# William-wAng618/roboticAttack

Hardware: AMD Instinct MI355X
Metric: attack-steps/sec (bs=64, 3x50x50 patch, OpenVLA-7B) (higher is better)
Workload: dtype bf16; 1 GPU; UADA_wrapper_ddp inner step: bs=64/rank (global 64), patch 3,50,50, geometry=True, maskidx=[0]; OpenVLA-7B shape, random init; u8 frames resident in HBM; global_batch=64, parallelism=dp1, regions=weak, visible_gpus=1, labelled_rows_per_rank=128, tunableop_entries_loaded_min_over_ranks=173

## Files before the change

include/vaa_model_ops.h:

```cpp
#ifndef VAA_MODEL_OPS_H_
#define VAA_MODEL_OPS_H_
#include <stdint.h>
#ifdef __cplusplus
extern "C" {
#endif
int vaa_model_rope(const uint16_t* x, long sb, long st, long sh, const float* cos_t, const float* sin_t, int B, int T, int H, int hd,
                   float sin_sign, uint16_t* out, void* stream);
int vaa_model_swiglu_fwd(const uint16_t* gate, const uint16_t* up, uint16_t* y, long n, void* stream);
int vaa_model_swiglu_bwd(const uint16_t* dy, const uint16_t* gate, const uint16_t* up, uint16_t* dgate, uint16_t* dup, long n, void* stream);
int vaa_model_scale_add(const uint16_t* x, const uint16_t* a, const uint16_t* ls, uint16_t* out, long rows, int D, void* stream);
int vaa_model_rmsnorm_fwd(const uint16_t* x, const uint16_t* w, uint16_t* h, float* rstd, long rows, int D, float eps, void* stream);
int vaa_model_rmsnorm_bwd(const uint16_t* gh, const uint16_t* gpass, const uint16_t* x, const uint16_t* w, const float* rstd, uint16_t* gx,
                          long rows, int D, void* stream);
int vaa_model_layernorm_fwd(const uint16_t* x, const uint16_t* w, const uint16_t* b, uint16_t* h, float* stats, long rows, int D, float eps,
                            void* stream);
int vaa_model_layernorm_bwd(const uint16_t* gh, const uint16_t* gpass, const uint16_t* x, const uint16_t* w, const float* stats, uint16_t* gx,
                            long rows, int D, void* stream);
int vaa_model_attention_fwd(const uint16_t* q, const int64_t* q_str, const uint16_t* k, const int64_t* k_str, const uint16_t* v,
                            const int64_t* v_str, uint16_t* o, const int64_t* o_str, float* lse, const int32_t* cu_seqlens, int B, int H,
                            int T, int hd, int causal, float scale, void* stream);
int vaa_model_attention_bwd(const uint16_t* q, const int64_t* q_str, const uint16_t* k, const int64_t* k_str, const uint16_t* v,
                            const int64_t* v_str, const uint16_t* o, const int64_t* o_str, const uint16_t* dout, const int64_t* do_str,
                            const float* lse, float* dsum, uint16_t* dq, const int64_t* dq_str, uint16_t* dk, const int64_t* dk_str,
                            uint16_t* dv, const int64_t* dv_str, const float* rope_cos, const float* rope_sin, const int32_t* cu_seqlens, int B,
                            int H, int T, int hd, int causal, float scale, void* stream);
#ifdef __cplusplus
}
#endif
#endif
```

roboticattack_amd/_lib.py:

```python
from __future__ import annotations

import ctypes as C
import os

_HERE = os.path.dirname(os.path.abspath(__file__))
LIB_PATH = os.environ.get("VAA_LIB_PATH") or os.path.join(_HERE, "libvaa_hip.so")

VAA_OK = 0
MASK_LT_M20, MASK_NE_M100 = 0, 1
LOSS_UADA, LOSS_UADA_DDP, LOSS_UPA, LOSS_CE = 0, 1, 2, 3
DTYPE_F32, DTYPE_BF16 = 0, 1
LAYOUT_FULL, LAYOUT_ROWS = 0, 1
GRAD_FULL, GRAD_SLICE = 0, 1
OPT_ADAMW_HF, OPT_PGD_SIGN = 0, 1

MODEL_OP_EXPORTS = ("vaa_model_rope", "vaa_model_swiglu_fwd", "vaa_model_swiglu_bwd", "vaa_model_rmsnorm_fwd", "vaa_model_rmsnorm_bwd",
                    "vaa_model_attention_fwd", "vaa_model_attention_bwd", "vaa_model_layernorm_fwd", "vaa_model_layernorm_bwd", "vaa_model_scale_add")

EXPORTS = (
    "vaa_last_error",
    "vaa_version",
    "vaa_device_check",
    "vaa_patch_apply_fwd",
    "vaa_patch_grad_ws_bytes",
    "vaa_patch_grad_gather",
    "vaa_loss_ws_bytes",
    "vaa_loss_fwd_bwd",
    "vaa_loss_fwd_bwd_ex",
    "vaa_patch_update",
    "vaa_patch_apply_eval",
    "vaa_patch_embed_grad_ws_bytes",
    "vaa_patch_embed_grad_gather",
    "vaa_patch_embed_packed_elems",
    "vaa_patch_embed_pack_weights",
    "vaa_patch_embed_grad_multi_ws_bytes",
    "vaa_patch_embed_grad_gather_multi",
    "vaa_patch_resize_fwd",
    "vaa_patch_resize_ws_bytes",
    "vaa_patch_resize_bwd",
    "vaa_patch_apply_fwd_multi",
    "vaa_patch_grad_gather_multi",
    "vaa_loss_rowmap_bytes",
    "vaa_loss_rowmap_build",
    "vaa_loss_rows_ws_bytes",
    "vaa_loss_rows_fwd_bwd",
    "vaa_patch_apply_fwd_tiles",
    "vaa_patch_grad_partials",
    "vaa_patch_embed_grad_gather_multi_tiles",
    "vaa_patch_embed_grad_gather_tiles",
    "vaa_loss_rows_stats",
    "vaa_head_loss_ws_bytes",
    "vaa_head_loss_rows_applies",
    "vaa_head_loss_rows_stats",
    "vaa_head_loss_rows_finish",
    "vaa_head_slice_applies",
    "vaa_head_slice_ws_bytes",
    "vaa_head_slice_pack",
    "vaa_head_slice_fwd_bwd",
    "vaa_step_epilogue",
    "vaa_step_epilogue_update",
    "vaa_loss_rowmap_seg_bytes",
    "vaa_loss_rowmap_build_seg",
    "vaa_step_epilogue_seg",
    "vaa_step_epilogue_seg_update",
    "vaa_patch_update_seg",
    "vaa_async_error",
    "vaa_prof_start",
    "vaa_prof_stop",
    "vaa_prof_get",
)


class VaaError(RuntimeError):
    pass


_lib = None


def _up_to_date() -> bool:
    if not os.path.exists(LIB_PATH):
        return False
    t = os.path.getmtime(LIB_PATH)
    src = os.path.join(_HERE, "csrc")
    deps = [os.path.join(src, f) for f in os.listdir(src)] + [os.path.join(_HERE, "..", "include", f) for f in ("vaa.h", "vaa_model_ops.h")]
    return all(os.path.getmtime(d) <= t for d in deps if os.path.exists(d))


def build(verbose: bool = False, force: bool = True) -> str:
    import fcntl
    import subprocess

    script = os.path.join(_HERE, "csrc", "build.sh")
    with open(os.path.join(_HERE, ".build.lock"), "w") as lock:
        fcntl.flock(lock, fcntl.LOCK_EX)
        try:
            if not force and _up_to_date():
                return LIB_PATH
            out = subprocess.run(["bash", script], capture_output=True, text=True)
        finally:
            fcntl.flock(lock, fcntl.LOCK_UN)
    if out.returncode != 0:
        raise VaaError(f"building libvaa_hip.so failed:\n{out.stdout}\n{out.stderr}")
    if verbose:
        print(out.stdout.strip())
    return LIB_PATH


def lib() -> C.CDLL:
    global _lib
    if _lib is not None:
        return _lib
    if not os.path.exists(LIB_PATH) and not os.environ.get("VAA_LIB_PATH") and os.path.exists(os.environ.get("HIPCC", "/opt/rocm/bin/hipcc")):
        build(force=False)
    if not os.path.exists(LIB_PATH):
        raise VaaError(
            f"{LIB_PATH} not found: the HIP extension is required (no CPU fallback). "
            "Build it with `python -c 'import __graft_entry__ as g; g.build()'` or roboticattack_amd/csrc/build.sh"
        )
    try:
        import torch
    except Exception:
        pass
    L = C.CDLL(LIB_PATH)
    vp, i32, f32, sz = C.c_void_p, C.c_int, C.c_float, C.c_size_t
    L.vaa_last_error.restype = C.c_char_p
    L.vaa_last_error.argtypes = []
    L.vaa_version.restype = i32
    L.vaa_device_check.restype = i32
    L.vaa_patch_apply_fwd.restype = i32
    L.vaa_patch_apply_fwd.argtypes = [vp, vp, vp, vp, i32, i32, i32, i32, i32, C.POINTER(f32), C.POINTER(f32), vp, vp, vp]
    L.vaa_patch_grad_ws_bytes.restype = sz
    L.vaa_patch_grad_ws_bytes.argtypes = [i32, i32, i32]
    L.vaa_patch_grad_gather.restype = i32
    L.vaa_patch_grad_gather.argtypes = [vp, vp, vp, vp, vp, i32, i32, i32, i32, i32, C.POINTER(f32), vp, vp, sz, vp]
    L.vaa_patch_embed_grad_ws_bytes.restype = sz
    L.vaa_patch_embed_grad_ws_bytes.argtypes = [i32, i32, i32]
    L.vaa_patch_embed_packed_elems.restype = sz
    L.vaa_patch_embed_packed_elems.argtypes = [i32]
    L.vaa_patch_embed_pack_weights.restype = i32
    L.vaa_patch_embed_pack_weights.argtypes = [vp, i32, vp, vp]
    L.vaa_patch_embed_grad_gather.restype = i32
    L.vaa_patch_embed_grad_gather.argtypes = [vp, i32, vp, i32, vp, vp, vp, vp, vp, vp, i32, i32, i32, i32, i32, C.POINTER(f32), i32, vp, vp, sz, vp]
    L.vaa_patch_embed_grad_multi_ws_bytes.restype = sz
    L.vaa_patch_embed_grad_multi_ws_bytes.argtypes = [i32]
    L.vaa_patch_embed_grad_gather_multi.restype = i32
    L.vaa_patch_embed_grad_gather_multi.argtypes = [vp, i32, vp, i32, vp, vp, vp, vp, vp, vp, vp, i32, i32, i32, i32, i32, C.POINTER(f32), i32, vp, vp, sz, vp]
    L.vaa_patch_resize_fwd.restype = i32
    L.vaa_patch_resize_fwd.argtypes = [vp, i32, i32, vp, i32, vp, vp]
    L.vaa_patch_resize_ws_bytes.restype = sz
    L.vaa_patch_resize_ws_bytes.argtypes = [i32, i32, i32]
    L.vaa_patch_resize_bwd.restype = i32
    L.vaa_patch_resize_bwd.argtypes = [vp, i32, i32, vp, i32, vp, vp, sz, vp]
    L.vaa_patch_apply_fwd_multi.restype = i32
    L.vaa_patch_apply_fwd_multi.argtypes = [vp, vp, vp, vp, vp, i32, i32, i32, i32, i32, C.POINTER(f32), C.POINTER(f32), vp, vp, vp]
    L.vaa_patch_grad_gather_multi.restype = i32
    L.vaa_patch_grad_gather_multi.argtypes = [vp, vp, vp, vp, vp, vp, i32, i32, i32, i32, i32, C.POINTER(f32), vp, vp]
    L.vaa_loss_ws_bytes.restype = sz
    L.vaa_loss_ws_bytes.argtypes = [i32, i32]
    L.vaa_loss_fwd_bwd.restype = i32
    L.vaa_loss_fwd_bwd.argtypes = [vp, i32, i32, vp, i32, i32, i32, i32, i32, C.POINTER(f32), vp, vp, vp, vp, sz, vp]
    L.vaa_loss_fwd_bwd_ex.restype = i32
    L.vaa_loss_fwd_bwd_ex.argtypes = [vp, i32, i32, vp, i32, i32, i32, i32, i32, C.POINTER(f32), vp, vp, vp, vp, vp, sz, vp]
    L.vaa_loss_rowmap_bytes.restype = sz
    L.vaa_loss_rowmap_bytes.argtypes = [i32, i32]
    L.vaa_loss_rowmap_build.restype = i32
    L.vaa_loss_rowmap_build.argtypes = [vp, i32, i32, vp, sz, vp]
    L.vaa_loss_rows_ws_bytes.restype = sz
    L.vaa_loss_rows_ws_bytes.argtypes = [i32]
    L.vaa_loss_rows_fwd_bwd.restype = i32
    L.vaa_loss_rows_fwd_bwd.argtypes = [vp, i32, vp, i32, i32, i32, i32, i32, C.POINTER(f32), vp, vp, vp, vp, i32, vp, sz, vp]
    L.vaa_patch_update.restype = i32
    L.vaa_patch_update.argtypes = [vp, vp, vp, vp, i32, i32, f32, f32, f32, f32, i32, f32, f32, vp, vp]
    L.vaa_patch_apply_eval.restype = i32
    L.vaa_patch_apply_eval.argtypes = [vp, vp, vp, vp, vp, i32, i32, i32, vp, vp]
    L.vaa_patch_apply_fwd_tiles.restype = i32
    L.vaa_patch_apply_fwd_tiles.argtypes = [vp, vp, vp, vp, vp, i32, i32, i32, i32, i32, C.POINTER(f32), C.POINTER(f32), vp, vp, vp, vp, vp]
    L.vaa_patch_embed_grad_gather_multi_tiles.restype = i32
    L.vaa_patch_embed_grad_gather_multi_tiles.argtypes = [vp, i32, vp, i32, vp, vp, vp, vp, vp, vp, vp, vp, i32, i32, i32, i32, i32, C.POINTER(f32), i32, vp, vp, sz, vp]
    L.vaa_patch_grad_partials.restype = i32
    L.vaa_patch_grad_partials.argtypes = [i32]
    L.vaa_patch_embed_grad_gather_tiles.restype = i32
    L.vaa_patch_embed_grad_gather_tiles.argtypes = [vp, i32, vp, i32, vp, vp, vp, vp, vp, vp, vp, i32, i32, i32, i32, i32, C.POINTER(f32), i32, vp, vp, sz, vp]
    L.vaa_loss_rows_stats.restype = i32
    L.vaa_loss_rows_stats.argtypes = [vp, i32, vp, i32, i32, i32, i32, i32, C.POINTER(f32), vp, i32, vp, sz, vp]
    L.vaa_head_loss_ws_bytes.restype = sz
    L.vaa_head_loss_ws_bytes.argtypes = [i32, i32]
    L.vaa_head_loss_rows_applies.restype = i32
    L.vaa_head_loss_rows_applies.argtypes = [i32, i32, i32]
    L.vaa_head_loss_rows_stats.restype = i32
    L.vaa_head_loss_rows_stats.argtypes = [vp, vp, i32, vp, i32, i32, i32, i32, i32, C.POINTER(f32), vp, vp, sz, vp, sz, vp, vp]
    L.vaa_head_loss_rows_finish.restype = i32
    L.vaa_head_loss_rows_finish.argtypes = [vp, i32, i32, i32, i32, i32, C.POINTER(f32), vp, sz, vp, sz, vp, vp, vp, vp, vp]
    L.vaa_head_slice_applies.restype = i32
    L.vaa_head_slice_applies.argtypes = [i32, i32, i32]
    L.vaa_head_slice_ws_bytes.restype = sz
    L.vaa_head_slice_ws_bytes.argtypes = [i32]
    L.vaa_head_slice_pack.restype = i32
    L.vaa_head_slice_pack.argtypes = [vp, i32, i32, vp, vp]
    L.vaa_head_slice_fwd_bwd.restype = i32
    L.vaa_head_slice_fwd_bwd.argtypes = [vp, vp, vp, i32, vp, i32, i32, i32, i32, i32, C.POINTER(f32), vp, vp, vp, sz, vp, vp, vp, vp, sz, vp]
    L.vaa_step_epilogue.restype = i32
    L.vaa_step_epilogue.argtypes = [vp, i32, i32, vp, i32, i32, i32, i32, i32, C.POINTER(f32), vp, sz, vp, vp, vp, vp, vp]
    L.vaa_step_epilogue_update.restype = i32
    L.vaa_step_epilogue_update.argtypes = [vp, i32, i32, vp, i32, i32, i32, i32, i32, C.POINTER(f32), vp, sz, vp, vp, vp, vp, vp, vp, vp, i32, f32, f32, f32, f32,
                                           i32, vp, vp]
    L.vaa_loss_rowmap_seg_bytes.restype = sz
    L.vaa_loss_rowmap_seg_bytes.argtypes = [i32, i32, i32]
    L.vaa_loss_rowmap_build_seg.restype = i32
    L.vaa_loss_rowmap_build_seg.argtypes = [vp, i32, i32, i32, vp, sz, vp]
    L.vaa_step_epilogue_seg.restype = i32
    L.vaa_step_epilogue_seg.argtypes = [vp, i32, i32, i32, vp, i32, i32, i32, i32, i32, C.POINTER(f32), vp, sz, vp, vp, vp, vp, vp]
    L.vaa_step_epilogue_seg_update.restype = i32
    L.vaa_step_epilogue_seg_update.argtypes = [vp, i32, i32, i32, vp, i32, i32, i32, i32, i32, C.POINTER(f32), vp, sz, vp, vp, vp, vp, vp, vp, vp, i32, f32,
                                               f32, f32, f32, i32, vp, vp]
    L.vaa_patch_update_seg.restype = i32
    L.vaa_patch_update_seg.argtypes = [vp, vp, vp, vp, i32, i32, i32, f32, f32, f32, f32, i32, f32, f32, vp, vp]
    L.vaa_async_error.restype = i32
    L.vaa_async_error.argtypes = []
    L.vaa_prof_start.restype = i32
    L.vaa_prof_start.argtypes = [i32]
    L.vaa_prof_stop.restype = i32
    L.vaa_prof_stop.argtypes = []
    L.vaa_prof_get.restype = i32
    L.vaa_prof_get.argtypes = [i32, C.POINTER(C.c_char_p), C.POINTER(f32)]
    lng = C.c_long
    L.vaa_model_rope.restype = i32
    L.vaa_model_rope.argtypes = [vp, lng, lng, lng, vp, vp, i32, i32, i32, i32, f32, vp, vp]
    L.vaa_model_swiglu_fwd.restype = i32
    L.vaa_model_swiglu_fwd.argtypes = [vp, vp, vp, lng, vp]
    L.vaa_model_swiglu_bwd.restype = i32
    L.vaa_model_swiglu_bwd.argtypes = [vp, vp, vp, vp, vp, lng, vp]
    L.vaa_model_scale_add.restype = i32
    L.vaa_model_scale_add.argtypes = [vp, vp, vp, vp, lng, i32, vp]
    L.vaa_model_rmsnorm_fwd.restype = i32
    L.vaa_model_rmsnorm_fwd.argtypes = [vp, vp, vp, vp, lng, i32, f32, vp]
    L.vaa_model_rmsnorm_bwd.restype = i32
    L.vaa_model_rmsnorm_bwd.argtypes = [vp, vp, vp, vp, vp, vp, lng, i32, vp]
    L.vaa_model_layernorm_fwd.restype = i32
    L.vaa_model_layernorm_fwd.argtypes = [vp, vp, vp, vp, vp, lng, i32, f32, vp]
    L.vaa_model_layernorm_bwd.restype = i32
    L.vaa_model_layernorm_bwd.argtypes = [vp, vp, vp, vp, vp, vp, lng, i32, vp]
    i64p = C.POINTER(C.c_int64)
    L.vaa_model_attention_fwd.restype = i32
    L.vaa_model_attention_fwd.argtypes = [vp, i64p, vp, i64p, vp, i64p, vp, i64p, vp, vp, i32, i32, i32, i32, i32, f32, vp]
    L.vaa_model_attention_bwd.restype = i32
    L.vaa_model_attention_bwd.argtypes = [vp, i64p, vp, i64p, vp, i64p, vp, i64p, vp, i64p, vp, vp, vp, i64p, vp, i64p, vp, i64p, vp, vp, vp, i32, i32, i32, i32, i32, f32, vp]
    _lib = L
    return L


def check(rc: int, what: str) -> None:
    if rc != VAA_OK:
        msg = lib().vaa_last_error().decode("utf-8", "replace")
        raise VaaError(f"{what} failed with code {rc}: {msg}")


def f32x(vals):
    return (C.c_float * len(vals))(*[float(v) for v in vals])
```

roboticattack_amd/csrc/vaa_attention.hip:

```cpp
#include "vaa_common.h"

#include <cstdlib>
#include <mutex>

#include "../../include/vaa_model_ops.h"

namespace vaa {

typedef short v4s __attribute__((ext_vector_type(4)));
typedef short v8s __attribute__((ext_vector_type(8)));
typedef float v4f __attribute__((ext_vector_type(4)));
typedef __attribute__((address_space(3))) v4s* lds_v4s_ptr;

struct AttnStr {
    long b, t, h;
};

struct AttnFwdArgs {
    const uint16_t *q, *k, *v;
    uint16_t* o;
    float* lse;
    AttnStr sq, sk, sv, so;
    const int32_t* cu;
    int B, H, T, hd;
    float scale_log2;
};

struct SeqInfo {
    int T;
    long tok0;
    bool packed;
};
__device__ __forceinline__ SeqInfo seq_info(const int32_t* cu, int b, int Tmax) {
    SeqInfo si;
    si.packed = cu != nullptr;
    si.tok0 = si.packed ? cu[b] : 0;
    si.T = si.packed ? cu[b + 1] - cu[b] : Tmax;
    return si;
}
__device__ __forceinline__ long row_base(const AttnStr& st, const SeqInfo& si, int b, int h) {
    return (si.packed ? si.tok0 * st.t : (long)b * st.b) + (long)h * st.h;
}

constexpr int kTile = 64;

__device__ __forceinline__ float fast_exp2(float x) { return __builtin_amdgcn_exp2f(x); }

__device__ __forceinline__ v4s lds_tr16(const uint16_t* p) {
    return __builtin_amdgcn_ds_read_tr16_b64_v4i16((lds_v4s_ptr)(p));
}

__device__ __forceinline__ v8s cat8(v4s lo, v4s hi) { return __builtin_shufflevector(lo, hi, 0, 1, 2, 3, 4, 5, 6, 7); }

typedef __bf16 bf2 __attribute__((ext_vector_type(2)));
typedef float f2 __attribute__((ext_vector_type(2)));

__device__ __forceinline__ uint32_t cvt_pk_bf16(float lo, float hi) {
    const bf2 r = __builtin_convertvector((f2){lo, hi}, bf2);
    return *reinterpret_cast<const uint32_t*>(&r);
}

__device__ __forceinline__ v8s pack8(v4f a, v4f b) {
    uint4 r;
    r.x = cvt_pk_bf16(a[0], a[1]);
    r.y = cvt_pk_bf16(a[2], a[3]);
    r.z = cvt_pk_bf16(b[0], b[1]);
    r.w = cvt_pk_bf16(b[2], b[3]);
    return *reinterpret_cast<v8s*>(&r);
}

typedef unsigned int v4u __attribute__((ext_vector_type(4)));

__device__ __forceinline__ __amdgpu_buffer_rsrc_t slice_rsrc(const uint16_t* base, long st, int T, int hd) {
    return __builtin_amdgcn_make_buffer_rsrc((void*)base, 0, (int)((((long)T - 1) * st + hd) * 2), 0x00020000);
}

template <int HDP>
struct TileRegs {
    static constexpr int kChunks = kTile * (HDP / 8) / 256;
    v4u r[kChunks];
    __device__ __forceinline__ void load(__amdgpu_buffer_rsrc_t rs, int st_bytes, int row0) {
#pragma unroll
        for (int it = 0; it < kChunks; ++it) {
            const int ch = threadIdx.x + it * 256;
            const int row = ch / (HDP / 8), cc = ch % (HDP / 8);
            r[it] = __builtin_amdgcn_raw_buffer_load_b128(rs, (row0 + row) * st_bytes + cc * 16, 0, 0);
        }
    }
    __device__ __forceinline__ void store(uint16_t* lds, int stride) const {
#pragma unroll
        for (int it = 0; it < kChunks; ++it) {
            const int ch = threadIdx.x + it * 256;
            const int row = ch / (HDP / 8), cc = ch % (HDP / 8);
            *reinterpret_cast<v4u*>(lds + row * stride + cc * 8) = r[it];
        }
    }
};

__device__ __forceinline__ bool block_to_pair(int nblk, int npairs, int& pair, int& blk, bool late_first = true) {
    const int bid = blockIdx.x, xcd = bid & 7, slot = bid >> 3;
    pair = (slot / nblk) * 8 + xcd;
    blk = late_first ? nblk - 1 - (slot % nblk) : slot % nblk;
    return pair < npairs;
}

template <int KS, int NT, bool CAUSAL, int G>
__global__ __launch_bounds__(256) void attn_fwd_kernel(AttnFwdArgs a) {
    constexpr int HDP = KS * 32;
    constexpr int SK = HDP + 8;
    constexpr int SV = HDP + 16;
    constexpr int QB = kTile * G, QW = 16 * G;
    __shared__ __attribute__((aligned(16))) uint16_t sK[kTile * SK];
    __shared__ __attribute__((aligned(16))) uint16_t sV[kTile * SV];

    const int nqb = (a.T + QB - 1) / QB;
    int pair, qb;
    if (!block_to_pair(nqb, a.B * a.H, pair, qb)) return;
    const int b = pair / a.H, h = pair - b * a.H;
    const SeqInfo si = seq_info(a.cu, b, a.T);
    const int T = si.T;
    if (qb * QB >= T) return;
    const int tid = threadIdx.x, lane = tid & 63, wv = tid >> 6, c = lane & 15, g = lane >> 4;
    const int q0 = qb * QB + wv * QW;

    const uint16_t* qp = a.q + row_base(a.sq, si, b, h);
    const uint16_t* kp = a.k + row_base(a.sk, si, b, h);
    const uint16_t* vp = a.v + row_base(a.sv, si, b, h);

    v8s qf[G][KS];
#pragma unroll
    for (int j = 0; j < G; ++j) {
        const int q = q0 + 16 * j + c;
#pragma unroll
        for (int ks = 0; ks < KS; ++ks) {
            const int d0 = ks * 32 + g * 8;
            uint4 r = make_uint4(0, 0, 0, 0);
            if (q < T && d0 < a.hd) r = *reinterpret_cast<const uint4*>(qp + (long)q * a.sq.t + d0);
            qf[j][ks] = *reinterpret_cast<v8s*>(&r);
        }
    }

    const int kend = CAUSAL ? min(T, (qb + 1) * QB) : T;
    const int ntile = (kend + kTile - 1) / kTile;

    v4f acc[G][NT];
    float m[G], lsum[G];
#pragma unroll
    for (int j = 0; j < G; ++j) {
#pragma unroll
        for (int nt = 0; nt < NT; ++nt) acc[j][nt] = (v4f){0.f, 0.f, 0.f, 0.f};
        m[j] = -INFINITY;
        lsum[j] = 0.0f;
    }

    const __amdgpu_buffer_rsrc_t krs = slice_rsrc(kp, a.sk.t, T, a.hd), vrs = slice_rsrc(vp, a.sv.t, T, a.hd);
    const int kst = (int)a.sk.t * 2, vst = (int)a.sv.t * 2;
    TileRegs<HDP> rk, rv;
    rk.load(krs, kst, 0);
    rv.load(vrs, vst, 0);
    for (int kt = 0; kt < ntile; ++kt) {
        __syncthreads();
        rk.store(sK, SK);
        rv.store(sV, SV);
        __syncthreads();
        if (kt + 1 < ntile) {
            rk.load(krs, kst, (kt + 1) * kTile);
            rv.load(vrs, vst, (kt + 1) * kTile);
        }
        const int key0 = kt * kTile;
        if (CAUSAL && key0 > q0 + QW - 1) continue;

        v4f st[G][4];
#pragma unroll
        for (int rp = 0; rp < 2; ++rp) {
            v8s kfr[2][KS];
#pragma unroll
            for (int rl = 0; rl < 2; ++rl)
#pragma unroll
                for (int ks = 0; ks < KS; ++ks) kfr[rl][ks] = *reinterpret_cast<const v8s*>(&sK[((2 * rp + rl) * 16 + c) * SK + ks * 32 + g * 8]);
#pragma unroll
            for (int j = 0; j < G; ++j)
#pragma unroll
                for (int rl = 0; rl < 2; ++rl) {
                    v4f t = (v4f){0.f, 0.f, 0.f, 0.f};
#pragma unroll
                    for (int ks = 0; ks < KS; ++ks) t = __builtin_amdgcn_mfma_f32_16x16x32_bf16(kfr[rl][ks], qf[j][ks], t, 0, 0, 0);
                    st[j][2 * rp + rl] = t;
                }
        }
#pragma unroll
        for (int j = 0; j < G; ++j) {
            const int qj0 = q0 + 16 * j, q = qj0 + c;
            const bool need_mask = (key0 + kTile > T) || (CAUSAL && key0 + kTile - 1 > qj0);
            if (need_mask) {
#pragma unroll
                for (int rt = 0; rt < 4; ++rt)
#pragma unroll
                    for (int r = 0; r < 4; ++r) {
                        const int key = key0 + rt * 16 + g * 4 + r;
                        if (key >= T || (CAUSAL && key > q)) st[j][rt][r] = -INFINITY;
                    }
            }
            float mx = -INFINITY;
#pragma unroll
            for (int rt = 0; rt < 4; ++rt)
#pragma unroll
                for (int r = 0; r < 4; ++r) mx = fmaxf(mx, st[j][rt][r]);
            mx = fmaxf(mx, __shfl_xor(mx, 16, 64));
            mx = fmaxf(mx, __shfl_xor(mx, 32, 64));
            const float mn = fmaxf(m[j], mx * a.scale_log2);
            const float mu = (mn == -INFINITY) ? 0.0f : mn;
            const float alpha = fast_exp2(m[j] - mu);
            m[j] = mn;
            float ps = 0.0f;
#pragma unroll
            for (int rt = 0; rt < 4; ++rt)
#pragma unroll
                for (int r = 0; r < 4; ++r) {
                    const float p = fast_exp2(__builtin_fmaf(st[j][rt][r], a.scale_log2, -mu));
                    st[j][rt][r] = p;
                    ps += p;
                }
            lsum[j] = lsum[j] * alpha + ps;
#pragma unroll
            for (int nt = 0; nt < NT; ++nt) acc[j][nt] *= alpha;
        }
#pragma unroll
        for (int half = 0; half < 2; ++half) {
            const uint16_t* vrow = &sV[(half * 32 + 4 * g + (c >> 2)) * SV + (c & 3) * 4];
            v8s vfr[NT];
#pragma unroll
            for (int nt = 0; nt < NT; ++nt) vfr[nt] = cat8(lds_tr16(vrow + nt * 16), lds_tr16(vrow + 16 * SV + nt * 16));
#pragma unroll
            for (int j = 0; j < G; ++j) {
                const v8s pf = pack8(st[j][2 * half], st[j][2 * half + 1]);
#pragma unroll
                for (int nt = 0; nt < NT; ++nt) acc[j][nt] = __builtin_amdgcn_mfma_f32_16x16x32_bf16(vfr[nt], pf, acc[j][nt], 0, 0, 0);
            }
        }
    }
#pragma unroll
    for (int j = 0; j < G; ++j) {
        const int q = q0 + 16 * j + c;
        float ls = lsum[j];
        ls += __shfl_xor(ls, 16, 64);
        ls += __shfl_xor(ls, 32, 64);
        if (q < T) {
            const float inv = ls > 0.0f ? 1.0f / ls : 0.0f;
            uint16_t* op = a.o + row_base(a.so, si, b, h) + (long)q * a.so.t;
#pragma unroll
            for (int nt = 0; nt < NT; ++nt) {
                const int d0 = nt * 16 + g * 4;
                if (d0 < a.hd) {
                    uint2 w;
                    w.x = cvt_pk_bf16(acc[j][nt][0] * inv, acc[j][nt][1] * inv);
                    w.y = cvt_pk_bf16(acc[j][nt][2] * inv, acc[j][nt][3] * inv);
                    *reinterpret_cast<uint2*>(op + d0) = w;
                }
            }
            if (g == 0) a.lse[((long)b * a.H + h) * a.T + q] = (m[j] + __builtin_log2f(ls)) * 0.69314718055994531f;
        }
    }
}

struct AttnBwdArgs {
    const uint16_t *q, *k, *v, *o, *dout;
    const float* lse;
    float* dsum;
    uint16_t *dq, *dk, *dv;
    AttnStr sq, sk, sv, so, sdo, sdq, sdk, sdv;
    const int32_t* cu;
    const float *rope_cos, *rope_sin;
    int B, H, T, hd;
    float scale, scale_log2;
};

template <int NT>
__device__ __forceinline__ void store_grad_row(uint16_t* op, const v4f (&acc)[NT], float scale, int g, int hd, const float* cosr, const float* sinr) {
    if (cosr) {
#pragma unroll
        for (int nt = 0; nt < NT / 2; ++nt) {
            const int d0 = nt * 16 + g * 4;
            const float4 c4 = *reinterpret_cast<const float4*>(cosr + d0), s4 = *reinterpret_cast<const float4*>(sinr + d0);
            const float cs[4] = {c4.x, c4.y, c4.z, c4.w}, sn[4] = {s4.x, s4.y, s4.z, s4.w};
            float o1[4], o2[4];
#pragma unroll
            for (int r = 0; r < 4; ++r) {
                const float g1 = acc[nt][r] * scale, g2 = acc[nt + NT / 2][r] * scale;
                o1[r] = g1 * cs[r] + g2 * sn[r];
                o2[r] = g2 * cs[r] - g1 * sn[r];
            }
            uint2 w;
            w.x = cvt_pk_bf16(o1[0], o1[1]); w.y = cvt_pk_bf16(o1[2], o1[3]);
            *reinterpret_cast<uint2*>(op + d0) = w;
            w.x = cvt_pk_bf16(o2[0], o2[1]); w.y = cvt_pk_bf16(o2[2], o2[3]);
            *reinterpret_cast<uint2*>(op + d0 + NT * 8) = w;
        }
        return;
    }
#pragma unroll
    for (int nt = 0; nt < NT; ++nt) {
        const int d0 = nt * 16 + g * 4;
        if (d0 < hd) {
            uint2 w;
            w.x = cvt_pk_bf16(acc[nt][0] * scale, acc[nt][1] * scale);
            w.y = cvt_pk_bf16(acc[nt][2] * scale, acc[nt][3] * scale);
            *reinterpret_cast<uint2*>(op + d0) = w;
        }
    }
}

template <int KS>
__device__ __forceinline__ void load_row_frags(v8s (&f)[KS], const uint16_t* row, bool valid, int g, int hd) {
#pragma unroll
    for (int ks = 0; ks < KS; ++ks) {
        const int d0 = ks * 32 + g * 8;
        uint4 r = make_uint4(0, 0, 0, 0);
        if (valid && d0 < hd) r = *reinterpret_cast<const uint4*>(row + d0);
        f[ks] = *reinterpret_cast<v8s*>(&r);
    }
}

__device__ __forceinline__ float bf_lo(uint32_t w) { return __uint_as_float(w << 16); }
__device__ __forceinline__ float bf_hi(uint32_t w) { return __uint_as_float(w & 0xffff0000u); }

template <int KS>
__device__ __forceinline__ void load_tile_frags(v8s (&af)[KS], const uint16_t* tile, int stride, int rt, int c, int g) {
#pragma unroll
    for (int ks = 0; ks < KS; ++ks) af[ks] = *reinterpret_cast<const v8s*>(&tile[(rt * 16 + c) * stride + ks * 32 + g * 8]);
}
template <int KS>
__device__ __forceinline__ v4f frag_dot(const v8s (&af)[KS], const v8s (&bf)[KS]) {
    v4f acc = (v4f){0.f, 0.f, 0.f, 0.f};
#pragma unroll
    for (int ks = 0; ks < KS; ++ks) acc = __builtin_amdgcn_mfma_f32_16x16x32_bf16(af[ks], bf[ks], acc, 0, 0, 0);
    return acc;
}

template <int KS, int NT, bool CAUSAL, int G>
__global__ __launch_bounds__(256) void attn_bwd_dq_kernel(AttnBwdArgs a) {
    constexpr int HDP = KS * 32;
    constexpr int SK = HDP + 16, SV = HDP + 8;
    constexpr int QB = kTile * G, QW = 16 * G;
    __shared__ __attribute__((aligned(16))) uint16_t sK[kTile * SK];
    __shared__ __attribute__((aligned(16))) uint16_t sV[kTile * SV];

    const int nqb = (a.T + QB - 1) / QB;
    int pair, qb;
    if (!block_to_pair(nqb, a.B * a.H, pair, qb)) return;
    const int b = pair / a.H, h = pair - b * a.H;
    const SeqInfo si = seq_info(a.cu, b, a.T);
    const int T = si.T;
    if (qb * QB >= T) return;
    const int tid = threadIdx.x, lane = tid & 63, wv = tid >> 6, c = lane & 15, g = lane >> 4;
    const int q0 = qb * QB + wv * QW;

    const uint16_t* kp = a.k + row_base(a.sk, si, b, h);
    const uint16_t* vp = a.v + row_base(a.sv, si, b, h);
    v8s qf[G][KS], dof[G][KS];
    float Dq[G], lse2[G];
#pragma unroll
    for (int j = 0; j < G; ++j) {
        const int q = q0 + 16 * j + c;
        const bool qv = q < T;
        load_row_frags<KS>(qf[j], a.q + row_base(a.sq, si, b, h) + (long)q * a.sq.t, qv, g, a.hd);
        load_row_frags<KS>(dof[j], a.dout + row_base(a.sdo, si, b, h) + (long)q * a.sdo.t, qv, g, a.hd);
        float dq_ = 0.0f;
        v8s of[KS];
        load_row_frags<KS>(of, a.o + row_base(a.so, si, b, h) + (long)q * a.so.t, qv, g, a.hd);
#pragma unroll
        for (int ks = 0; ks < KS; ++ks)
#pragma unroll
            for (int e = 0; e < 8; ++e) dq_ += bf16_bits_to_f32((uint16_t)of[ks][e]) * bf16_bits_to_f32((uint16_t)dof[j][ks][e]);
        dq_ += __shfl_xor(dq_, 16, 64);
        dq_ += __shfl_xor(dq_, 32, 64);
        Dq[j] = dq_;
        const long rowid = ((long)b * a.H + h) * a.T + q;
        if (qv && g == 0) a.dsum[rowid] = dq_;
        lse2[j] = qv ? a.lse[rowid] * 1.4426950408889634f : INFINITY;
    }

    const int kend = CAUSAL ? min(T, (qb + 1) * QB) : T;
    const int ntile = (kend + kTile - 1) / kTile;
    v4f acc[G][NT];
#pragma unroll
    for (int j = 0; j < G; ++j)
#pragma unroll
        for (int nt = 0; nt < NT; ++nt) acc[j][nt] = (v4f){0.f, 0.f, 0.f, 0.f};

    const __amdgpu_buffer_rsrc_t krs = slice_rsrc(kp, a.sk.t, T, a.hd), vrs = slice_rsrc(vp, a.sv.t, T, a.hd);
    const int kst = (int)a.sk.t * 2, vst = (int)a.sv.t * 2;
    TileRegs<HDP> rk, rv;
    rk.load(krs, kst, 0);
    rv.load(vrs, vst, 0);
    for (int kt = 0; kt < ntile; ++kt) {
        __syncthreads();
        rk.store(sK, SK);
        rv.store(sV, SV);
        __syncthreads();
        if (kt + 1 < ntile) {
            rk.load(krs, kst, (kt + 1) * kTile);
            rv.load(vrs, vst, (kt + 1) * kTile);
        }
        const int key0 = kt * kTile;
        if (CAUSAL && key0 > q0 + QW - 1) continue;
        const bool need_mask = (key0 + kTile > T) || (CAUSAL && key0 + kTile - 1 > q0);
#pragma unroll
        for (int half = 0; half < 2; ++half) {
            if (CAUSAL && key0 + half * 32 > q0 + QW - 1) continue;
            v4f ds[G][2];
#pragma unroll
            for (int rl = 0; rl < 2; ++rl) {
                const int rt = 2 * half + rl;
                v8s ak[KS], av[KS];
                load_tile_frags<KS>(ak, sK, SK, rt, c, g);
                load_tile_frags<KS>(av, sV, SV, rt, c, g);
#pragma unroll
                for (int j = 0; j < G; ++j) {
                    const v4f st = frag_dot<KS>(ak, qf[j]);
                    const v4f dp = frag_dot<KS>(av, dof[j]);
                    const int q = q0 + 16 * j + c;
#pragma unroll
                    for (int r = 0; r < 4; ++r) {
                        float p = fast_exp2(__builtin_fmaf(st[r], a.scale_log2, -lse2[j]));
                        if (need_mask) {
                            const int key = key0 + rt * 16 + g * 4 + r;
                            if (key >= T || (CAUSAL && key > q)) p = 0.0f;
                        }
                        ds[j][rl][r] = p * (dp[r] - Dq[j]);
                    }
                }
            }
            const uint16_t* krow = &sK[(half * 32 + 4 * g + (c >> 2)) * SK + (c & 3) * 4];
            v8s kfr[NT];
#pragma unroll
            for (int nt = 0; nt < NT; ++nt) kfr[nt] = cat8(lds_tr16(krow + nt * 16), lds_tr16(krow + 16 * SK + nt * 16));
#pragma unroll
            for (int j = 0; j < G; ++j) {
                const v8s dsf = pack8(ds[j][0], ds[j][1]);
#pragma unroll
                for (int nt = 0; nt < NT; ++nt) acc[j][nt] = __builtin_amdgcn_mfma_f32_16x16x32_bf16(kfr[nt], dsf, acc[j][nt], 0, 0, 0);
            }
        }
    }
#pragma unroll
    for (int j = 0; j < G; ++j) {
        const int q = q0 + 16 * j + c;
        if (q < T) {
            const long ro = (si.tok0 + q) * (a.hd >> 1);
            store_grad_row<NT>(a.dq + row_base(a.sdq, si, b, h) + (long)q * a.sdq.t, acc[j], a.scale, g, a.hd,
                               a.rope_cos ? a.rope_cos + ro : nullptr, a.rope_cos ? a.rope_sin + ro : nullptr);
        }
    }
}

template <int KS, int NT, bool CAUSAL, int G>
__global__ __launch_bounds__(256) void attn_bwd_dkv_kernel(AttnBwdArgs a) {
    constexpr int HDP = KS * 32;
    constexpr int SQ = HDP + 16;
    constexpr int KB = kTile * G, KW = 16 * G;
    __shared__ __attribute__((aligned(16))) uint16_t sQ[kTile * SQ];
    __shared__ __attribute__((aligned(16))) uint16_t sDO[kTile * SQ];
    __shared__ float sL[kTile], sD[kTile];

    const int nkb = (a.T + KB - 1) / KB;
    int pair, kb;
    if (!block_to_pair(nkb, a.B * a.H, pair, kb, !CAUSAL)) return;
    const int b = pair / a.H, h = pair - b * a.H;
    const SeqInfo si = seq_info(a.cu, b, a.T);
    const int T = si.T;
    if (kb * KB >= T) return;
    const int tid = threadIdx.x, lane = tid & 63, wv = tid >> 6, c = lane & 15, g = lane >> 4;
    const int key0w = kb * KB + wv * KW;

    v8s kf[G][KS], vf[G][KS];
#pragma unroll
    for (int j = 0; j < G; ++j) {
        const int key = key0w + 16 * j + c;
        load_row_frags<KS>(kf[j], a.k + row_base(a.sk, si, b, h) + (long)key * a.sk.t, key < T, g, a.hd);
        load_row_frags<KS>(vf[j], a.v + row_base(a.sv, si, b, h) + (long)key * a.sv.t, key < T, g, a.hd);
    }
    const uint16_t* qp = a.q + row_base(a.sq, si, b, h);
    const uint16_t* dop = a.dout + row_base(a.sdo, si, b, h);
    const float* lsep = a.lse + ((long)b * a.H + h) * a.T;
    const float* dsp = a.dsum + ((long)b * a.H + h) * a.T;

    v4f dk[G][NT], dv[G][NT];
#pragma unroll
    for (int j = 0; j < G; ++j)
#pragma unroll
        for (int nt = 0; nt < NT; ++nt) {
            dk[j][nt] = (v4f){0.f, 0.f, 0.f, 0.f};
            dv[j][nt] = (v4f){0.f, 0.f, 0.f, 0.f};
        }
    const int nqt = (T + kTile - 1) / kTile;
    const int qt0 = CAUSAL ? kb * G : 0;
    TileRegs<HDP> rq, rdo;
    float rstat = 0.0f;
    auto load_stats = [&](int qbase) {
        if (tid < 128) {
            const int qq = qbase + (tid & 63);
            if (tid < 64) rstat = qq < T ? lsep[qq] * 1.4426950408889634f : INFINITY;
            else rstat = qq < T ? dsp[qq] : 0.0f;
        }
    };
    const __amdgpu_buffer_rsrc_t qrs = slice_rsrc(qp, a.sq.t, T, a.hd), dors = slice_rsrc(dop, a.sdo.t, T, a.hd);
    const int qst = (int)a.sq.t * 2, dost = (int)a.sdo.t * 2;
    rq.load(qrs, qst, qt0 * kTile);
    rdo.load(dors, dost, qt0 * kTile);
    load_stats(qt0 * kTile);
    for (int qt = qt0; qt < nqt; ++qt) {
        __syncthreads();
        rq.store(sQ, SQ);
        rdo.store(sDO, SQ);
        if (tid < 64) sL[tid] = rstat;
        else if (tid < 128) sD[tid - 64] = rstat;
        __syncthreads();
        if (qt + 1 < nqt) {
            rq.load(qrs, qst, (qt + 1) * kTile);
            rdo.load(dors, dost, (qt + 1) * kTile);
            load_stats((qt + 1) * kTile);
        }
        const int qb0 = qt * kTile;
        if (CAUSAL && qb0 + kTile - 1 < key0w) continue;
        const bool need_mask = CAUSAL && qb0 < key0w + KW - 1;
#pragma unroll
        for (int half = 0; half < 2; ++half) {
            if (CAUSAL && qb0 + half * 32 + 31 < key0w) continue;
            v4f p[G][2], ds[G][2];
#pragma unroll
            for (int rl = 0; rl < 2; ++rl) {
                const int rt = 2 * half + rl;
                v8s aq[KS], ado[KS];
                load_tile_frags<KS>(aq, sQ, SQ, rt, c, g);
                load_tile_frags<KS>(ado, sDO, SQ, rt, c, g);
#pragma unroll
                for (int j = 0; j < G; ++j) {
                    const v4f s = frag_dot<KS>(aq, kf[j]);
                    const v4f dp = frag_dot<KS>(ado, vf[j]);
                    const int key = key0w + 16 * j + c;
#pragma unroll
                    for (int r = 0; r < 4; ++r) {
                        const int ql = rt * 16 + g * 4 + r;
                        float pe = fast_exp2(__builtin_fmaf(s[r], a.scale_log2, -sL[ql]));
                        if (CAUSAL && need_mask && key > qb0 + ql) pe = 0.0f;
                        p[j][rl][r] = pe;
                        ds[j][rl][r] = pe * (dp[r] - sD[ql]);
                    }
                }
            }
            const int ro = (half * 32 + 4 * g + (c >> 2)) * SQ + (c & 3) * 4;
            {
                v8s fr[NT];
#pragma unroll
                for (int nt = 0; nt < NT; ++nt) fr[nt] = cat8(lds_tr16(&sDO[ro + nt * 16]), lds_tr16(&sDO[ro + 16 * SQ + nt * 16]));
#pragma unroll
                for (int j = 0; j < G; ++j) {
                    const v8s pf = pack8(p[j][0], p[j][1]);
#pragma unroll
                    for (int nt = 0; nt < NT; ++nt) dv[j][nt] = __builtin_amdgcn_mfma_f32_16x16x32_bf16(fr[nt], pf, dv[j][nt], 0, 0, 0);
                }
#pragma unroll
                for (int nt = 0; nt < NT; ++nt) fr[nt] = cat8(lds_tr16(&sQ[ro + nt * 16]), lds_tr16(&sQ[ro + 16 * SQ + nt * 16]));
#pragma unroll
                for (int j = 0; j < G; ++j) {
                    const v8s dsf = pack8(ds[j][0], ds[j][1]);
#pragma unroll
                    for (int nt = 0; nt < NT; ++nt) dk[j][nt] = __builtin_amdgcn_mfma_f32_16x16x32_bf16(fr[nt], dsf, dk[j][nt], 0, 0, 0);
                }
            }
        }
    }
#pragma unroll
    for (int j = 0; j < G; ++j) {
        const int key = key0w + 16 * j + c;
        if (key < T) {
            const long ro = (si.tok0 + key) * (a.hd >> 1);
            store_grad_row<NT>(a.dk + row_base(a.sdk, si, b, h) + (long)key * a.sdk.t, dk[j], a.scale, g, a.hd,
                               a.rope_cos ? a.rope_cos + ro : nullptr, a.rope_cos ? a.rope_sin + ro : nullptr);
            store_grad_row<NT>(a.dv + row_base(a.sdv, si, b, h) + (long)key * a.sdv.t, dv[j], 1.0f, g, a.hd, nullptr, nullptr);
        }
    }
}

static void attn_groups(int hd, int& gf, int& gq, int& gk) {
    static int cfg[3] = {0, 0, 0};
    static std::once_flag once;
    std::call_once(once, [] {
        const char* ev = getenv("VAA_ATTN_G");
        for (int i = 0; i < 3; ++i) cfg[i] = (ev && ev[0] && ev[1] && ev[2] && (ev[i] == '1' || ev[i] == '2')) ? ev[i] - '0' : 0;
    });
    const int dflt = (hd > 64 && hd <= 80) ? 2 : 1;
    gf = cfg[0] ? cfg[0] : dflt;
    gq = cfg[1] ? cfg[1] : dflt;
    gk = cfg[2] ? cfg[2] : dflt;
}

template <bool CAUSAL>
static int launch_bwd(const AttnBwdArgs& a, hipStream_t st) {
    int gf, gq, gk;
    attn_groups(a.hd, gf, gq, gk);
    const unsigned pairs8 = (unsigned)(((long)a.B * a.H + 7) / 8 * 8);
    const unsigned grid_q = pairs8 * (unsigned)((a.T + kTile * gq - 1) / (kTile * gq)), grid_k = pairs8 * (unsigned)((a.T + kTile * gk - 1) / (kTile * gk));
#define VAA_ATT_BWD(KS, NT)                                                                                                  \
    do {                                                                                                                     \
        if (gq == 2) hipLaunchKernelGGL((attn_bwd_dq_kernel<KS, NT, CAUSAL, 2>), dim3(grid_q), dim3(256), 0, st, a);         \
        else hipLaunchKernelGGL((attn_bwd_dq_kernel<KS, NT, CAUSAL, 1>), dim3(grid_q), dim3(256), 0, st, a);                 \
        int rc = check_launch("vaa_model_attention_bwd(dq)");                                                                \
        if (rc != VAA_OK) return rc;                                                                                         \
        if (gk == 2) hipLaunchKernelGGL((attn_bwd_dkv_kernel<KS, NT, CAUSAL, 2>), dim3(grid_k), dim3(256), 0, st, a);        \
        else hipLaunchKernelGGL((attn_bwd_dkv_kernel<KS, NT, CAUSAL, 1>), dim3(grid_k), dim3(256), 0, st, a);                \
        return check_launch("vaa_model_attention_bwd(dkv)");                                                                 \
    } while (0)
    if (a.hd <= 64) VAA_ATT_BWD(2, 4);
    else if (a.hd <= 80) VAA_ATT_BWD(3, 5);
    else if (a.hd <= 96) VAA_ATT_BWD(3, 6);
    else VAA_ATT_BWD(4, 8);
#undef VAA_ATT_BWD
}

template <bool CAUSAL>
static int launch_fwd(const AttnFwdArgs& a, hipStream_t st) {
    int gf, gq, gk;
    attn_groups(a.hd, gf, gq, gk);
    const unsigned grid = (unsigned)(((long)a.B * a.H + 7) / 8 * 8) * (unsigned)((a.T + kTile * gf - 1) / (kTile * gf));
#define VAA_ATT_FWD(KS, NT)                                                                                          \
    do {                                                                                                             \
        if (gf == 2) hipLaunchKernelGGL((attn_fwd_kernel<KS, NT, CAUSAL, 2>), dim3(grid), dim3(256), 0, st, a);      \
        else hipLaunchKernelGGL((attn_fwd_kernel<KS, NT, CAUSAL, 1>), dim3(grid), dim3(256), 0, st, a);              \
    } while (0)
    if (a.hd <= 64) VAA_ATT_FWD(2, 4);
    else if (a.hd <= 80) VAA_ATT_FWD(3, 5);
    else if (a.hd <= 96) VAA_ATT_FWD(3, 6);
    else VAA_ATT_FWD(4, 8);
#undef VAA_ATT_FWD
    return check_launch("vaa_model_attention_fwd");
}

static bool strides_ok(const int64_t* s) { return s && (s[0] % 8) == 0 && (s[1] % 8) == 0 && (s[2] % 8) == 0; }
static AttnStr mk(const int64_t* s) { AttnStr r; r.b = s[0]; r.t = s[1]; r.h = s[2]; return r; }

}

extern "C" int vaa_model_attention_fwd(const uint16_t* q, const int64_t* q_str, const uint16_t* k, const int64_t* k_str, const uint16_t* v,
                                       const int64_t* v_str, uint16_t* o, const int64_t* o_str, float* lse, const int32_t* cu_seqlens, int B,
                                       int H, int T, int hd, int causal, float scale, void* stream) {
    using namespace vaa;
    if (!q || !k || !v || !o || !lse) {
        set_error("vaa_model_attention_fwd: null pointer argument");
        return VAA_E_INVALID;
    }
    if (B <= 0 || H <= 0 || T <= 0 || hd <= 0 || hd > 128 || (hd % 8) != 0 || !strides_ok(q_str) || !strides_ok(k_str) || !strides_ok(v_str) ||
        !strides_ok(o_str)) {
        set_error("vaa_model_attention_fwd: unsupported shape (B=%d H=%d T=%d hd=%d; hd %% 8 == 0, hd <= 128, strides %% 8 == 0)", B, H, T, hd);
        return VAA_E_UNSUPPORTED;
    }
    AttnFwdArgs a;
    a.q = q; a.k = k; a.v = v; a.o = o; a.lse = lse;
    a.sq = mk(q_str); a.sk = mk(k_str); a.sv = mk(v_str); a.so = mk(o_str);
    a.cu = cu_seqlens;
    a.B = B; a.H = H; a.T = T; a.hd = hd;
    a.scale_log2 = scale * 1.4426950408889634f;
    return causal ? launch_fwd<true>(a, (hipStream_t)stream) : launch_fwd<false>(a, (hipStream_t)stream);
}

extern "C" int vaa_model_attention_bwd(const uint16_t* q, const int64_t* q_str, const uint16_t* k, const int64_t* k_str, const uint16_t* v,
                                       const int64_t* v_str, const uint16_t* o, const int64_t* o_str, const uint16_t* dout,
                                       const int64_t* do_str, const float* lse, float* dsum, uint16_t* dq, const int64_t* dq_str, uint16_t* dk,
                                       const int64_t* dk_str, uint16_t* dv, const int64_t* dv_str, const float* rope_cos, const float* rope_sin,
                                       const int32_t* cu_seqlens, int B, int H, int T, int hd, int causal, float scale, void* stream) {
    using namespace vaa;
    if (!q || !k || !v || !o || !dout || !lse || !dsum || !dq || !dk || !dv) {
        set_error("vaa_model_attention_bwd: null pointer argument");
        return VAA_E_INVALID;
    }
    if (B <= 0 || H <= 0 || T <= 0 || hd <= 0 || hd > 128 || (hd % 8) != 0 || !strides_ok(q_str) || !strides_ok(k_str) || !strides_ok(v_str) ||
        !strides_ok(o_str) || !strides_ok(do_str) || !strides_ok(dq_str) || !strides_ok(dk_str) || !strides_ok(dv_str)) {
        set_error("vaa_model_attention_bwd: unsupported shape (B=%d H=%d T=%d hd=%d; hd %% 8 == 0, hd <= 128, strides %% 8 == 0)", B, H, T, hd);
        return VAA_E_UNSUPPORTED;
    }
    AttnBwdArgs a;
    a.q = q; a.k = k; a.v = v; a.o = o; a.dout = dout; a.lse = lse; a.dsum = dsum; a.dq = dq; a.dk = dk; a.dv = dv;
    a.sq = mk(q_str); a.sk = mk(k_str); a.sv = mk(v_str); a.so = mk(o_str); a.sdo = mk(do_str);
    a.sdq = mk(dq_str); a.sdk = mk(dk_str); a.sdv = mk(dv_str);
    if ((rope_cos != nullptr) != (rope_sin != nullptr) || (rope_cos && hd != 64 && hd != 128)) {
        set_error("vaa_model_attention_bwd: fused rotary adjoint needs both tables and hd in {64, 128} (hd=%d)", hd);
        return VAA_E_UNSUPPORTED;
    }
    a.rope_cos = rope_cos; a.rope_sin = rope_sin;
    a.cu = cu_seqlens;
    a.B = B; a.H = H; a.T = T; a.hd = hd;
    a.scale = scale;
    a.scale_log2 = scale * 1.4426950408889634f;
    return causal ? launch_bwd<true>(a, (hipStream_t)stream) : launch_bwd<false>(a, (hipStream_t)stream);
}
```

roboticattack_amd/model_ops.py:

```python
from __future__ import annotations

import os

import torch

from . import _lib


def enabled(x: torch.Tensor) -> bool:
    return x.is_cuda and x.dtype == torch.bfloat16 and not os.environ.get("VAA_NO_FUSED_MODEL_OPS")


def attention_enabled(x_bthd: torch.Tensor) -> bool:
    hd = x_bthd.shape[-1]
    return (enabled(x_bthd) and not os.environ.get("VAA_NO_FUSED_ATTENTION") and hd % 8 == 0 and hd <= 128
            and all(s % 8 == 0 for s in x_bthd.stride()[:-1]) and x_bthd.stride(-1) == 1)


def _stream():
    return torch.cuda.current_stream().cuda_stream


def _rope_launch(x_bthd: torch.Tensor, cos: torch.Tensor, sin: torch.Tensor, sign: float) -> torch.Tensor:
    B, T, H, hd = x_bthd.shape
    if x_bthd.stride(3) != 1:
        x_bthd = x_bthd.contiguous()
    out = torch.empty((B, T, H, hd), dtype=torch.bfloat16, device=x_bthd.device)
    rc = _lib.lib().vaa_model_rope(x_bthd.data_ptr(), x_bthd.stride(0), x_bthd.stride(1), x_bthd.stride(2), cos.data_ptr(), sin.data_ptr(),
                                   B, T, H, hd, float(sign), out.data_ptr(), _stream())
    _lib.check(rc, "vaa_model_rope")
    return out


class RopeFn(torch.autograd.Function):

    @staticmethod
    def forward(ctx, x, cos, sin):
        ctx.save_for_backward(cos, sin)
        return _rope_launch(x, cos, sin, 1.0)

    @staticmethod
    def backward(ctx, g):
        cos, sin = ctx.saved_tensors
        return _rope_launch(g, cos, sin, -1.0), None, None


class SwiGLUFn(torch.autograd.Function):

    @staticmethod
    def forward(ctx, gate, up):
        gate, up = gate.contiguous(), up.contiguous()
        y = torch.empty_like(gate)
        _lib.check(_lib.lib().vaa_model_swiglu_fwd(gate.data_ptr(), up.data_ptr(), y.data_ptr(), gate.numel(), _stream()), "vaa_model_swiglu_fwd")
        ctx.save_for_backward(gate, up)
        return y

    @staticmethod
    def backward(ctx, dy):
        gate, up = ctx.saved_tensors
        dy = dy.contiguous()
        dg, du = torch.empty_like(gate), torch.empty_like(up)
        _lib.check(_lib.lib().vaa_model_swiglu_bwd(dy.data_ptr(), gate.data_ptr(), up.data_ptr(), dg.data_ptr(), du.data_ptr(), gate.numel(), _stream()),
                   "vaa_model_swiglu_bwd")
        return dg, du


def _scale_add(x, a, ls):
    D = a.shape[-1]
    out = torch.empty_like(a)
    _lib.check(_lib.lib().vaa_model_scale_add(x.data_ptr() if x is not None else None, a.data_ptr(), ls.data_ptr(), out.data_ptr(), a.numel() // D, D,
                                              _stream()), "vaa_model_scale_add")
    return out


class ScaleAddFn(torch.autograd.Function):

    @staticmethod
    def forward(ctx, x, a, ls):
        ctx.save_for_backward(ls)
        return _scale_add(x.contiguous(), a.contiguous(), ls.contiguous())

    @staticmethod
    def backward(ctx, g):
        (ls,) = ctx.saved_tensors
        g = g.contiguous()
        da = _scale_add(None, g, ls.contiguous()) if ctx.needs_input_grad[1] else None
        return (g if ctx.needs_input_grad[0] else None), da, None


def scale_add(x: torch.Tensor, a: torch.Tensor, ls: torch.Tensor) -> torch.Tensor:
    if (enabled(x) and a.dtype == x.dtype and ls.dtype == x.dtype and x.shape == a.shape and ls.dim() == 1 and ls.shape[0] == x.shape[-1]
            and x.shape[-1] % 8 == 0 and a.device == x.device and ls.device == x.device and not ls.requires_grad
            and os.environ.get("VAA_MODEL_SCALE_ADD", "1") != "0"):
        return ScaleAddFn.apply(x, a, ls)
    return torch.addcmul(x, a, ls)


class ResidualRMSNormFn(torch.autograd.Function):

    @staticmethod
    def forward(ctx, x, weight, eps):
        x = x.contiguous()
        D = x.shape[-1]
        rows = x.numel() // D
        h = torch.empty_like(x)
        rstd = torch.empty(rows, dtype=torch.float32, device=x.device)
        _lib.check(_lib.lib().vaa_model_rmsnorm_fwd(x.data_ptr(), weight.data_ptr(), h.data_ptr(), rstd.data_ptr(), rows, D, float(eps), _stream()),
                   "vaa_model_rmsnorm_fwd")
        ctx.save_for_backward(x, weight, rstd)
        return x, h

    @staticmethod
    def backward(ctx, g_pass, g_h):
        x, weight, rstd = ctx.saved_tensors
        D = x.shape[-1]
        rows = x.numel() // D
        if g_h is None:
            return g_pass, None, None
        g_h = g_h.contiguous()
        gp = g_pass.contiguous() if g_pass is not None else None
        gx = torch.empty_like(x)
        _lib.check(_lib.lib().vaa_model_rmsnorm_bwd(g_h.data_ptr(), gp.data_ptr() if gp is not None else None, x.data_ptr(), weight.data_ptr(),
                                                    rstd.data_ptr(), gx.data_ptr(), rows, D, _stream()), "vaa_model_rmsnorm_bwd")
        return gx, None, None


class ResidualLayerNormFn(torch.autograd.Function):

    @staticmethod
    def forward(ctx, x, weight, bias, eps):
        x = x.contiguous()
        D = x.shape[-1]
        rows = x.numel() // D
        h = torch.empty_like(x)
        stats = torch.empty((rows, 2), dtype=torch.float32, device=x.device)
        _lib.check(_lib.lib().vaa_model_layernorm_fwd(x.data_ptr(), weight.data_ptr(), bias.data_ptr(), h.data_ptr(), stats.data_ptr(), rows, D,
                                                      float(eps), _stream()), "vaa_model_layernorm_fwd")
        ctx.save_for_backward(x, weight, stats)
        return x, h

    @staticmethod
    def backward(ctx, g_pass, g_h):
        x, weight, stats = ctx.saved_tensors
        D = x.shape[-1]
        rows = x.numel() // D
        if g_h is None:
            return g_pass, None, None, None
        g_h = g_h.contiguous()
        gp = g_pass.contiguous() if g_pass is not None else None
        gx = torch.empty_like(x)
        _lib.check(_lib.lib().vaa_model_layernorm_bwd(g_h.data_ptr(), gp.data_ptr() if gp is not None else None, x.data_ptr(), weight.data_ptr(),
                                                      stats.data_ptr(), gx.data_ptr(), rows, D, _stream()), "vaa_model_layernorm_bwd")
        return gx, None, None, None


def tn_dgrad_enabled() -> bool:
    return not os.environ.get("VAA_NO_TN_DGRAD")


class FrozenLinearsFn(torch.autograd.Function):

    @staticmethod
    def forward(ctx, x, res, *ws):
        x2 = x.reshape(-1, x.shape[-1])
        W, Wt = ws[0::2], ws[1::2]
        ctx.wt = Wt
        ctx.xshape = x.shape
        ctx.has_res = res is not None
        if res is not None:
            return (torch.addmm(res.reshape(-1, W[0].shape[0]), x2, W[0].t()).view(*x.shape[:-1], W[0].shape[0]),)
        return tuple(torch.nn.functional.linear(x2, w).view(*x.shape[:-1], w.shape[0]) for w in W)

    @staticmethod
    def backward(ctx, *dys):
        dx = None
        for dy, wt in zip(dys, ctx.wt):
            if dy is None:
                continue
            d2 = dy.reshape(-1, dy.shape[-1])
            if dx is None:
                dx = torch.nn.functional.linear(d2, wt)
            else:
                dx.addmm_(d2, wt.t())
        dx = dx.view(ctx.xshape) if dx is not None else None
        dres = dys[0] if ctx.has_res else None
        return (dx, dres) + (None,) * (2 * len(ctx.wt))


def _str3(x: torch.Tensor):
    import ctypes

    if x.stride(3) != 1:
        raise ValueError("attention operands need a contiguous head dimension")
    return (ctypes.c_int64 * 3)(x.stride(0), x.stride(1), x.stride(2))


def attention_fwd(q: torch.Tensor, k: torch.Tensor, v: torch.Tensor, causal: bool, scale: float | None = None, cu_seqlens=None, max_len: int = 0):
    Bq, T, H, hd = q.shape
    scale = float(hd) ** -0.5 if scale is None else float(scale)
    o = torch.empty((Bq, T, H, hd), dtype=torch.bfloat16, device=q.device)
    B, Tm = (int(cu_seqlens.numel()) - 1, int(max_len)) if cu_seqlens is not None else (Bq, T)
    lse = torch.empty((B, H, Tm), dtype=torch.float32, device=q.device)
    rc = _lib.lib().vaa_model_attention_fwd(q.data_ptr(), _str3(q), k.data_ptr(), _str3(k), v.data_ptr(), _str3(v), o.data_ptr(), _str3(o),
                                            lse.data_ptr(), cu_seqlens.data_ptr() if cu_seqlens is not None else None, B, H, Tm, hd,
                                            int(bool(causal)), scale, _stream())
    _lib.check(rc, "vaa_model_attention_fwd")
    return o, lse


def attention_bwd(q, k, v, o, lse, dout, causal: bool, scale: float, packed_grad: bool = False, rope=None, cu_seqlens=None, max_len: int = 0):
    Bq, T, H, hd = q.shape
    B, Tm = (int(cu_seqlens.numel()) - 1, int(max_len)) if cu_seqlens is not None else (Bq, T)
    if dout.stride(3) != 1:
        dout = dout.contiguous()
    if packed_grad:
        buf = torch.empty((Bq, T, 3, H, hd), dtype=torch.bfloat16, device=q.device)
        dq, dk, dv = buf[:, :, 0], buf[:, :, 1], buf[:, :, 2]
    else:
        buf = None
        dq, dk, dv = (torch.empty((Bq, T, H, hd), dtype=torch.bfloat16, device=q.device) for _ in range(3))
    dsum = torch.empty((B, H, Tm), dtype=torch.float32, device=q.device)
    rc = _lib.lib().vaa_model_attention_bwd(q.data_ptr(), _str3(q), k.data_ptr(), _str3(k), v.data_ptr(), _str3(v), o.data_ptr(), _str3(o),
                                            dout.data_ptr(), _str3(dout), lse.data_ptr(), dsum.data_ptr(), dq.data_ptr(), _str3(dq),
                                            dk.data_ptr(), _str3(dk), dv.data_ptr(), _str3(dv), rope[0].data_ptr() if rope else None,
                                            rope[1].data_ptr() if rope else None, cu_seqlens.data_ptr() if cu_seqlens is not None else None,
                                            B, H, Tm, hd, int(bool(causal)), float(scale), _stream())
    _lib.check(rc, "vaa_model_attention_bwd")
    return buf if packed_grad else (dq, dk, dv)


class AttentionFn(torch.autograd.Function):

    @staticmethod
    def forward(ctx, q, k, v, causal, scale):
        scale = float(q.shape[-1]) ** -0.5 if scale is None else float(scale)
        o, lse = attention_fwd(q, k, v, causal, scale)
        ctx.save_for_backward(q, k, v, o, lse)
        ctx.causal, ctx.scale = bool(causal), scale
        return o

    @staticmethod
    def backward(ctx, dout):
        q, k, v, o, lse = ctx.saved_tensors
        dq, dk, dv = attention_bwd(q, k, v, o, lse, dout, ctx.causal, ctx.scale)
        return dq, dk, dv, None, None


class RopeAttentionFn(torch.autograd.Function):

    @staticmethod
    def forward(ctx, q, k, v, cos, sin, causal, scale, cu_seqlens=None, max_len=0):
        scale = float(q.shape[-1]) ** -0.5 if scale is None else float(scale)
        qr, kr = _rope_launch(q, cos, sin, 1.0), _rope_launch(k, cos, sin, 1.0)
        o, lse = attention_fwd(qr, kr, v, causal, scale, cu_seqlens, max_len)
        ctx.save_for_backward(qr, kr, v, o, lse, cos, sin, *([cu_seqlens] if cu_seqlens is not None else []))
        ctx.causal, ctx.scale, ctx.max_len = bool(causal), scale, int(max_len)
        return o

    @staticmethod
    def backward(ctx, dout):
        qr, kr, v, o, lse, cos, sin, *cu = ctx.saved_tensors
        dq, dk, dv = attention_bwd(qr, kr, v, o, lse, dout, ctx.causal, ctx.scale, rope=(cos, sin), cu_seqlens=cu[0] if cu else None,
                                   max_len=ctx.max_len)
        return dq, dk, dv, None, None, None, None, None, None


class RopePackedAttentionFn(torch.autograd.Function):

    @staticmethod
    def forward(ctx, qkv, cos, sin, causal, scale, cu_seqlens=None, max_len=0):
        scale = float(qkv.shape[-1]) ** -0.5 if scale is None else float(scale)
        qr, kr = _rope_launch(qkv[:, :, 0], cos, sin, 1.0), _rope_launch(qkv[:, :, 1], cos, sin, 1.0)
        v = qkv[:, :, 2]
        o, lse = attention_fwd(qr, kr, v, causal, scale, cu_seqlens, max_len)
        ctx.save_for_backward(qr, kr, qkv, o, lse, cos, sin, *([cu_seqlens] if cu_seqlens is not None else []))
        ctx.causal, ctx.scale, ctx.max_len = bool(causal), scale, int(max_len)
        return o

    @staticmethod
    def backward(ctx, dout):
        qr, kr, qkv, o, lse, cos, sin, *cu = ctx.saved_tensors
        buf = attention_bwd(qr, kr, qkv[:, :, 2], o, lse, dout, ctx.causal, ctx.scale, packed_grad=True, rope=(cos, sin),
                            cu_seqlens=cu[0] if cu else None, max_len=ctx.max_len)
        return buf, None, None, None, None, None, None


class PackedAttentionFn(torch.autograd.Function):

    @staticmethod
    def forward(ctx, qkv, causal, scale):
        scale = float(qkv.shape[-1]) ** -0.5 if scale is None else float(scale)
        o, lse = attention_fwd(qkv[:, :, 0], qkv[:, :, 1], qkv[:, :, 2], causal, scale)
        ctx.save_for_backward(qkv, o, lse)
        ctx.causal, ctx.scale = bool(causal), scale
        return o

    @staticmethod
    def backward(ctx, dout):
        qkv, o, lse = ctx.saved_tensors
        return attention_bwd(qkv[:, :, 0], qkv[:, :, 1], qkv[:, :, 2], o, lse, dout, ctx.causal, ctx.scale, packed_grad=True), None, None
```

Before: 2.178 attack-steps/s.

## Fuse rotary embedding into attention kernels and add direct K/V tile staging

Adds rope-fused forward and backward attention entry points that rotate Q and K inside the flash kernels using the cos/sin tables. This removes the separate rope launches and the saved rotated Q/K copies, but it only runs when VAA_ATTN_FORM=rope_in is set. It also adds a 'direct' staging mode that loads each K/V (or Q/dO) tile just before use instead of prefetching the next tile in registers. Under the default form this mode is on for forward with head dim above 96 and for dK/dV with head dim 64 or below, and a waves-per-EU hint is added for the direct forward case. The trade is less register pressure and possibly higher occupancy against less load/compute overlap.

```diff
diff --git a/include/vaa_model_ops.h b/include/vaa_model_ops.h
--- a/include/vaa_model_ops.h
+++ b/include/vaa_model_ops.h
@@ -24,6 +24,16 @@
                             const float* lse, float* dsum, uint16_t* dq, const int64_t* dq_str, uint16_t* dk, const int64_t* dk_str,
                             uint16_t* dv, const int64_t* dv_str, const float* rope_cos, const float* rope_sin, const int32_t* cu_seqlens, int B,
                             int H, int T, int hd, int causal, float scale, void* stream);
+int vaa_model_attention_rope_fwd(const uint16_t* q, const int64_t* q_str, const uint16_t* k, const int64_t* k_str, const uint16_t* v,
+                                 const int64_t* v_str, uint16_t* o, const int64_t* o_str, float* lse, const float* rope_cos,
+                                 const float* rope_sin, const int32_t* cu_seqlens, int B, int H, int T, int hd, int causal, float scale,
+                                 void* stream);
+int vaa_model_attention_rope_bwd(const uint16_t* q, const int64_t* q_str, const uint16_t* k, const int64_t* k_str, const uint16_t* v,
+                                 const int64_t* v_str, const uint16_t* o, const int64_t* o_str, const uint16_t* dout, const int64_t* do_str,
+                                 const float* lse, float* dsum, uint16_t* dq, const int64_t* dq_str, uint16_t* dk, const int64_t* dk_str,
+                                 uint16_t* dv, const int64_t* dv_str, const float* rope_cos, const float* rope_sin, const int32_t* cu_seqlens,
+                                 int B, int H, int T, int hd, int causal, float scale, void* stream);
+int vaa_model_attention_form(int form);
 #ifdef __cplusplus
 }
 #endif
diff --git a/roboticattack_amd/_lib.py b/roboticattack_amd/_lib.py
--- a/roboticattack_amd/_lib.py
+++ b/roboticattack_amd/_lib.py
@@ -15,7 +15,8 @@
 OPT_ADAMW_HF, OPT_PGD_SIGN = 0, 1
 
 MODEL_OP_EXPORTS = ("vaa_model_rope", "vaa_model_swiglu_fwd", "vaa_model_swiglu_bwd", "vaa_model_rmsnorm_fwd", "vaa_model_rmsnorm_bwd",
-                    "vaa_model_attention_fwd", "vaa_model_attention_bwd", "vaa_model_layernorm_fwd", "vaa_model_layernorm_bwd", "vaa_model_scale_add")
+                    "vaa_model_attention_fwd", "vaa_model_attention_bwd", "vaa_model_layernorm_fwd", "vaa_model_layernorm_bwd", "vaa_model_scale_add",
+                    "vaa_model_attention_rope_fwd", "vaa_model_attention_rope_bwd", "vaa_model_attention_form")
 
 EXPORTS = (
     "vaa_last_error",
@@ -246,6 +247,12 @@
     L.vaa_model_attention_fwd.argtypes = [vp, i64p, vp, i64p, vp, i64p, vp, i64p, vp, vp, i32, i32, i32, i32, i32, f32, vp]
     L.vaa_model_attention_bwd.restype = i32
     L.vaa_model_attention_bwd.argtypes = [vp, i64p, vp, i64p, vp, i64p, vp, i64p, vp, i64p, vp, vp, vp, i64p, vp, i64p, vp, i64p, vp, vp, vp, i32, i32, i32, i32, i32, f32, vp]
+    L.vaa_model_attention_rope_fwd.restype = i32
+    L.vaa_model_attention_rope_fwd.argtypes = [vp, i64p, vp, i64p, vp, i64p, vp, i64p, vp, vp, vp, vp, i32, i32, i32, i32, i32, f32, vp]
+    L.vaa_model_attention_rope_bwd.restype = i32
+    L.vaa_model_attention_rope_bwd.argtypes = L.vaa_model_attention_bwd.argtypes
+    L.vaa_model_attention_form.restype = i32
+    L.vaa_model_attention_form.argtypes = [i32]
     _lib = L
     return L
 
diff --git a/roboticattack_amd/csrc/vaa_attention.hip b/roboticattack_amd/csrc/vaa_attention.hip
--- a/roboticattack_amd/csrc/vaa_attention.hip
+++ b/roboticattack_amd/csrc/vaa_attention.hip
@@ -1,6 +1,8 @@
 #include "vaa_common.h"
 
+#include <atomic>
 #include <cstdlib>
+#include <cstring>
 #include <mutex>
 
 #include "../../include/vaa_model_ops.h"
@@ -22,6 +24,7 @@
     float* lse;
     AttnStr sq, sk, sv, so;
     const int32_t* cu;
+    const float *rope_cos, *rope_sin;
     int B, H, T, hd;
     float scale_log2;
 };
@@ -75,27 +78,89 @@
     return __builtin_amdgcn_make_buffer_rsrc((void*)base, 0, (int)((((long)T - 1) * st + hd) * 2), 0x00020000);
 }
 
+__device__ __forceinline__ void rope8(v4u& lo, v4u& hi, v4u c0, v4u c1, v4u s0, v4u s1) {
+    const float cs[8] = {__uint_as_float(c0[0]), __uint_as_float(c0[1]), __uint_as_float(c0[2]), __uint_as_float(c0[3]),
+                         __uint_as_float(c1[0]), __uint_as_float(c1[1]), __uint_as_float(c1[2]), __uint_as_float(c1[3])};
+    const float sn[8] = {__uint_as_float(s0[0]), __uint_as_float(s0[1]), __uint_as_float(s0[2]), __uint_as_float(s0[3]),
+                         __uint_as_float(s1[0]), __uint_as_float(s1[1]), __uint_as_float(s1[2]), __uint_as_float(s1[3])};
+#pragma unroll
+    for (int q = 0; q < 4; ++q) {
+        const float x1a = __uint_as_float(lo[q] << 16), x1b = __uint_as_float(lo[q] & 0xffff0000u);
+        const float x2a = __uint_as_float(hi[q] << 16), x2b = __uint_as_float(hi[q] & 0xffff0000u);
+        const float o1a = x1a * cs[2 * q] - x2a * sn[2 * q], o1b = x1b * cs[2 * q + 1] - x2b * sn[2 * q + 1];
+        const float o2a = x2a * cs[2 * q] + x1a * sn[2 * q], o2b = x2b * cs[2 * q + 1] + x1b * sn[2 * q + 1];
+        lo[q] = f32_to_bf16_bits(o1a) | (f32_to_bf16_bits(o1b) << 16);
+        hi[q] = f32_to_bf16_bits(o2a) | (f32_to_bf16_bits(o2b) << 16);
+    }
+}
+
+template <int KS>
+__device__ __forceinline__ void rope_frags(v8s (&f)[KS], bool valid, const float* cosr, const float* sinr, int g) {
+    if (!valid) return;
+#pragma unroll
+    for (int ks = 0; ks < KS / 2; ++ks) {
+        v4u lo = *reinterpret_cast<v4u*>(&f[ks]), hi = *reinterpret_cast<v4u*>(&f[ks + KS / 2]);
+        const float *cp = cosr + ks * 32 + g * 8, *sp = sinr + ks * 32 + g * 8;
+        rope8(lo, hi, *reinterpret_cast<const v4u*>(cp), *reinterpret_cast<const v4u*>(cp + 4), *reinterpret_cast<const v4u*>(sp),
+              *reinterpret_cast<const v4u*>(sp + 4));
+        f[ks] = *reinterpret_cast<v8s*>(&lo);
+        f[ks + KS / 2] = *reinterpret_cast<v8s*>(&hi);
+    }
+}
+
+template <int HDP, bool PAIRED = false>
+struct TileRegs {
+    static constexpr int kCpr = HDP / 8;
+    static constexpr int kChunks = kTile * kCpr / 256;
+    v4u r[kChunks];
+    __device__ __forceinline__ static void place(int it, int& row, int& cc) {
+        if (PAIRED) {
+            const int pi = threadIdx.x + (it >> 1) * 256;
+            row = pi / (kCpr / 2);
+            cc = pi % (kCpr / 2) + (it & 1) * (kCpr / 2);
+        } else {
+            const int ch = threadIdx.x + it * 256;
+            row = ch / kCpr;
+            cc = ch % kCpr;
+        }
+    }
+    __device__ __forceinline__ void load(__amdgpu_buffer_rsrc_t rs, int st_bytes, int row0) {
+#pragma unroll
+        for (int it = 0; it < kChunks; ++it) {
+            int row, cc;
+            place(it, row, cc);
+            r[it] = __builtin_amdgcn_raw_buffer_load_b128(rs, (row0 + row) * st_bytes + cc * 16, 0, 0);
+        }
+    }
+    __device__ __forceinline__ void rotate(__amdgpu_buffer_rsrc_t crs, __amdgpu_buffer_rsrc_t srs, int row0) {
+        static_assert(PAIRED, "rotation needs both halves of a row in one thread");
+#pragma unroll
+        for (int i = 0; i < kChunks / 2; ++i) {
+            int row, cc;
+            place(2 * i, row, cc);
+            const int off = (row0 + row) * (HDP * 2) + cc * 32;
+            rope8(r[2 * i], r[2 * i + 1], __builtin_amdgcn_raw_buffer_load_b128(crs, off, 0, 0), __builtin_amdgcn_raw_buffer_load_b128(crs, off + 16, 0, 0),
+                  __builtin_amdgcn_raw_buffer_load_b128(srs, off, 0, 0), __builtin_amdgcn_raw_buffer_load_b128(srs, off + 16, 0, 0));
+            __builtin_amdgcn_sched_barrier(0);
+        }
+    }
+    __device__ __forceinline__ void store(uint16_t* lds, int stride) const {
+#pragma unroll
+        for (int it = 0; it < kChunks; ++it) {
+            int row, cc;
+            place(it, row, cc);
+            *reinterpret_cast<v4u*>(lds + row * stride + cc * 8) = r[it];
+        }
+    }
+};
+
 template <int HDP>
-struct TileRegs {
-    static constexpr int kChunks = kTile * (HDP / 8) / 256;
-    v4u r[kChunks];
-    __device__ __forceinline__ void load(__amdgpu_buffer_rsrc_t rs, int st_bytes, int row0) {
-#pragma unroll
-        for (int it = 0; it < kChunks; ++it) {
-            const int ch = threadIdx.x + it * 256;
-            const int row = ch / (HDP / 8), cc = ch % (HDP / 8);
-            r[it] = __builtin_amdgcn_raw_buffer_load_b128(rs, (row0 + row) * st_bytes + cc * 16, 0, 0);
-        }
-    }
-    __device__ __forceinline__ void store(uint16_t* lds, int stride) const {
-#pragma unroll
-        for (int it = 0; it < kChunks; ++it) {
-            const int ch = threadIdx.x + it * 256;
-            const int row = ch / (HDP / 8), cc = ch % (HDP / 8);
-            *reinterpret_cast<v4u*>(lds + row * stride + cc * 8) = r[it];
-        }
-    }
-};
+__device__ __forceinline__ __amdgpu_buffer_rsrc_t rope_rsrc(const float* tab, long tok0, int T) {
+    return __builtin_amdgcn_make_buffer_rsrc((void*)(tab + tok0 * (HDP / 2)), 0, T * (HDP * 2), 0x00020000);
+}
+
+enum { kStageReg = 0, kStageDirect = 1 };
+constexpr int fwd_waves(int G, int stage) { return (G == 1 && stage == kStageDirect) ? 4 : 1; }
 
 __device__ __forceinline__ bool block_to_pair(int nblk, int npairs, int& pair, int& blk, bool late_first = true) {
     const int bid = blockIdx.x, xcd = bid & 7, slot = bid >> 3;
@@ -104,8 +169,8 @@
     return pair < npairs;
 }
 
-template <int KS, int NT, bool CAUSAL, int G>
-__global__ __launch_bounds__(256) void attn_fwd_kernel(AttnFwdArgs a) {
+template <int KS, int NT, bool CAUSAL, int G, bool ROPE = false, int STAGE = kStageReg>
+__global__ __launch_bounds__(256) __attribute__((amdgpu_waves_per_eu(fwd_waves(G, STAGE)))) void attn_fwd_kernel(AttnFwdArgs a) {
     constexpr int HDP = KS * 32;
     constexpr int SK = HDP + 8;
     constexpr int SV = HDP + 16;
@@ -138,6 +203,10 @@
             if (q < T && d0 < a.hd) r = *reinterpret_cast<const uint4*>(qp + (long)q * a.sq.t + d0);
             qf[j][ks] = *reinterpret_cast<v8s*>(&r);
         }
+        if (ROPE) {
+            const long ro = (si.tok0 + q) * (HDP / 2);
+            rope_frags<KS>(qf[j], q < T, a.rope_cos + ro, a.rope_sin + ro, g);
+        }
     }
 
     const int kend = CAUSAL ? min(T, (qb + 1) * QB) : T;
@@ -155,15 +224,26 @@
 
     const __amdgpu_buffer_rsrc_t krs = slice_rsrc(kp, a.sk.t, T, a.hd), vrs = slice_rsrc(vp, a.sv.t, T, a.hd);
     const int kst = (int)a.sk.t * 2, vst = (int)a.sv.t * 2;
-    TileRegs<HDP> rk, rv;
-    rk.load(krs, kst, 0);
-    rv.load(vrs, vst, 0);
+    TileRegs<HDP, ROPE> rk;
+    TileRegs<HDP> rv;
+    if (STAGE == kStageReg) {
+        rk.load(krs, kst, 0);
+        rv.load(vrs, vst, 0);
+    }
     for (int kt = 0; kt < ntile; ++kt) {
         __syncthreads();
+        if (STAGE == kStageDirect) {
+            rk.load(krs, kst, kt * kTile);
+            rv.load(vrs, vst, kt * kTile);
+        }
+        rv.store(sV, SV);
+        if constexpr (ROPE) {
+            __builtin_amdgcn_sched_barrier(0);
+            rk.rotate(rope_rsrc<HDP>(a.rope_cos, si.tok0, T), rope_rsrc<HDP>(a.rope_sin, si.tok0, T), kt * kTile);
+        }
         rk.store(sK, SK);
-        rv.store(sV, SV);
         __syncthreads();
-        if (kt + 1 < ntile) {
+        if (STAGE == kStageReg && kt + 1 < ntile) {
             rk.load(krs, kst, (kt + 1) * kTile);
             rv.load(vrs, vst, (kt + 1) * kTile);
         }
@@ -337,7 +417,7 @@
     return acc;
 }
 
-template <int KS, int NT, bool CAUSAL, int G>
+template <int KS, int NT, bool CAUSAL, int G, bool ROPE = false, int STAGE = kStageReg>
 __global__ __launch_bounds__(256) void attn_bwd_dq_kernel(AttnBwdArgs a) {
     constexpr int HDP = KS * 32;
     constexpr int SK = HDP + 16, SV = HDP + 8;
@@ -364,6 +444,10 @@
         const int q = q0 + 16 * j + c;
         const bool qv = q < T;
         load_row_frags<KS>(qf[j], a.q + row_base(a.sq, si, b, h) + (long)q * a.sq.t, qv, g, a.hd);
+        if (ROPE) {
+            const long ro = (si.tok0 + q) * (HDP / 2);
+            rope_frags<KS>(qf[j], qv, a.rope_cos + ro, a.rope_sin + ro, g);
+        }
         load_row_frags<KS>(dof[j], a.dout + row_base(a.sdo, si, b, h) + (long)q * a.sdo.t, qv, g, a.hd);
         float dq_ = 0.0f;
         v8s of[KS];
@@ -390,15 +474,26 @@
 
     const __amdgpu_buffer_rsrc_t krs = slice_rsrc(kp, a.sk.t, T, a.hd), vrs = slice_rsrc(vp, a.sv.t, T, a.hd);
     const int kst = (int)a.sk.t * 2, vst = (int)a.sv.t * 2;
-    TileRegs<HDP> rk, rv;
-    rk.load(krs, kst, 0);
-    rv.load(vrs, vst, 0);
+    TileRegs<HDP, ROPE> rk;
+    TileRegs<HDP> rv;
+    if (STAGE == kStageReg) {
+        rk.load(krs, kst, 0);
+        rv.load(vrs, vst, 0);
+    }
     for (int kt = 0; kt < ntile; ++kt) {
         __syncthreads();
+        if (STAGE == kStageDirect) {
+            rk.load(krs, kst, kt * kTile);
+            rv.load(vrs, vst, kt * kTile);
+        }
+        rv.store(sV, SV);
+        if constexpr (ROPE) {
+            __builtin_amdgcn_sched_barrier(0);
+            rk.rotate(rope_rsrc<HDP>(a.rope_cos, si.tok0, T), rope_rsrc<HDP>(a.rope_sin, si.tok0, T), kt * kTile);
+        }
         rk.store(sK, SK);
-        rv.store(sV, SV);
         __syncthreads();
-        if (kt + 1 < ntile) {
+        if (STAGE == kStageReg && kt + 1 < ntile) {
             rk.load(krs, kst, (kt + 1) * kTile);
             rv.load(vrs, vst, (kt + 1) * kTile);
         }
@@ -454,7 +549,7 @@
     }
 }
 
-template <int KS, int NT, bool CAUSAL, int G>
+template <int KS, int NT, bool CAUSAL, int G, bool ROPE = false, int STAGE = kStageReg>
 __global__ __launch_bounds__(256) void attn_bwd_dkv_kernel(AttnBwdArgs a) {
     constexpr int HDP = KS * 32;
     constexpr int SQ = HDP + 16;
@@ -478,6 +573,10 @@
     for (int j = 0; j < G; ++j) {
         const int key = key0w + 16 * j + c;
         load_row_frags<KS>(kf[j], a.k + row_base(a.sk, si, b, h) + (long)key * a.sk.t, key < T, g, a.hd);
+        if (ROPE) {
+            const long ro = (si.tok0 + key) * (HDP / 2);
+            rope_frags<KS>(kf[j], key < T, a.rope_cos + ro, a.rope_sin + ro, g);
+        }
         load_row_frags<KS>(vf[j], a.v + row_base(a.sv, si, b, h) + (long)key * a.sv.t, key < T, g, a.hd);
     }
     const uint16_t* qp = a.q + row_base(a.sq, si, b, h);
@@ -495,7 +594,8 @@
         }
     const int nqt = (T + kTile - 1) / kTile;
     const int qt0 = CAUSAL ? kb * G : 0;
-    TileRegs<HDP> rq, rdo;
+    TileRegs<HDP, ROPE> rq;
+    TileRegs<HDP> rdo;
     float rstat = 0.0f;
     auto load_stats = [&](int qbase) {
         if (tid < 128) {
@@ -506,17 +606,28 @@
     };
     const __amdgpu_buffer_rsrc_t qrs = slice_rsrc(qp, a.sq.t, T, a.hd), dors = slice_rsrc(dop, a.sdo.t, T, a.hd);
     const int qst = (int)a.sq.t * 2, dost = (int)a.sdo.t * 2;
-    rq.load(qrs, qst, qt0 * kTile);
-    rdo.load(dors, dost, qt0 * kTile);
-    load_stats(qt0 * kTile);
+    if (STAGE == kStageReg) {
+        rq.load(qrs, qst, qt0 * kTile);
+        rdo.load(dors, dost, qt0 * kTile);
+        load_stats(qt0 * kTile);
+    }
     for (int qt = qt0; qt < nqt; ++qt) {
         __syncthreads();
+        if (STAGE == kStageDirect) {
+            rq.load(qrs, qst, qt * kTile);
+            rdo.load(dors, dost, qt * kTile);
+            load_stats(qt * kTile);
+        }
+        rdo.store(sDO, SQ);
+        if constexpr (ROPE) {
+            __builtin_amdgcn_sched_barrier(0);
+            rq.rotate(rope_rsrc<HDP>(a.rope_cos, si.tok0, T), rope_rsrc<HDP>(a.rope_sin, si.tok0, T), qt * kTile);
+        }
         rq.store(sQ, SQ);
-        rdo.store(sDO, SQ);
         if (tid < 64) sL[tid] = rstat;
         else if (tid < 128) sD[tid - 64] = rstat;
         __syncthreads();
-        if (qt + 1 < nqt) {
+        if (STAGE == kStageReg && qt + 1 < nqt) {
             rq.load(qrs, qst, (qt + 1) * kTile);
             rdo.load(dors, dost, (qt + 1) * kTile);
             load_stats((qt + 1) * kTile);
@@ -596,72 +707,177 @@
     gk = cfg[2] ? cfg[2] : dflt;
 }
 
-template <bool CAUSAL>
+enum { kFormTile64 = 0, kFormCurrent = 1, kFormRopeIn = 2 };
+static std::atomic<int>& attn_form() {
+    static std::atomic<int> form{[] {
+        const char* ev = getenv("VAA_ATTN_FORM");
+        if (ev && strcmp(ev, "tile64") == 0) return (int)kFormTile64;
+        if (ev && strcmp(ev, "rope_in") == 0) return (int)kFormRopeIn;
+        return (int)kFormCurrent;
+    }()};
+    return form;
+}
+
+static void attn_stages(int hd, int& sf, int& sq, int& sk) {
+    static int cfg[3] = {-1, -1, -1};
+    static std::once_flag once;
+    std::call_once(once, [] {
+        const char* ev = getenv("VAA_ATTN_STAGE");
+        for (int i = 0; i < 3; ++i)
+            cfg[i] = (ev && ev[0] && ev[1] && ev[2] && (ev[i] == 'r' || ev[i] == 'd')) ? (ev[i] == 'd' ? kStageDirect : kStageReg) : -1;
+    });
+    sf = sq = sk = kStageReg;
+    if (attn_form().load() == kFormTile64) return;
+    sf = cfg[0] >= 0 ? cfg[0] : (hd > 96 ? kStageDirect : kStageReg);
+    sq = cfg[1] >= 0 ? cfg[1] : kStageReg;
+    sk = cfg[2] >= 0 ? cfg[2] : (hd <= 64 ? kStageDirect : kStageReg);
+}
+
+#define VAA_ATT_PICK(KERNEL, KS, NT, G, STG, GRID, ARGS)                                                                                   \
+    do {                                                                                                                                   \
+        if (ROPE || G == 1) {                                                                                                              \
+            if (STG == kStageDirect) hipLaunchKernelGGL((KERNEL<KS, NT, CAUSAL, 1, ROPE, kStageDirect>), dim3(GRID), dim3(256), 0, st, ARGS); \
+            else hipLaunchKernelGGL((KERNEL<KS, NT, CAUSAL, 1, ROPE, kStageReg>), dim3(GRID), dim3(256), 0, st, ARGS);                      \
+        } else {                                                                                                                           \
+            if (STG == kStageDirect) hipLaunchKernelGGL((KERNEL<KS, NT, CAUSAL, 2, false, kStageDirect>), dim3(GRID), dim3(256), 0, st, ARGS); \
+            else hipLaunchKernelGGL((KERNEL<KS, NT, CAUSAL, 2, false, kStageReg>), dim3(GRID), dim3(256), 0, st, ARGS);                     \
+        }                                                                                                                                  \
+    } while (0)
+
+template <int KS, int NT, bool CAUSAL, bool ROPE>
+static int launch_bwd_t(const AttnBwdArgs& a, int gq, int gk, hipStream_t st) {
+    int sf, sq, sk;
+    attn_stages(a.hd, sf, sq, sk);
+    const unsigned pairs8 = (unsigned)(((long)a.B * a.H + 7) / 8 * 8);
+    const unsigned grid_q = pairs8 * (unsigned)((a.T + kTile * gq - 1) / (kTile * gq)), grid_k = pairs8 * (unsigned)((a.T + kTile * gk - 1) / (kTile * gk));
+    VAA_ATT_PICK(attn_bwd_dq_kernel, KS, NT, gq, sq, grid_q, a);
+    const int rc = check_launch("vaa_model_attention_bwd(dq)");
+    if (rc != VAA_OK) return rc;
+    VAA_ATT_PICK(attn_bwd_dkv_kernel, KS, NT, gk, sk, grid_k, a);
+    return check_launch("vaa_model_attention_bwd(dkv)");
+}
+
+template <bool CAUSAL, bool ROPE>
 static int launch_bwd(const AttnBwdArgs& a, hipStream_t st) {
     int gf, gq, gk;
     attn_groups(a.hd, gf, gq, gk);
-    const unsigned pairs8 = (unsigned)(((long)a.B * a.H + 7) / 8 * 8);
-    const unsigned grid_q = pairs8 * (unsigned)((a.T + kTile * gq - 1) / (kTile * gq)), grid_k = pairs8 * (unsigned)((a.T + kTile * gk - 1) / (kTile * gk));
-#define VAA_ATT_BWD(KS, NT)                                                                                                  \
-    do {                                                                                                                     \
-        if (gq == 2) hipLaunchKernelGGL((attn_bwd_dq_kernel<KS, NT, CAUSAL, 2>), dim3(grid_q), dim3(256), 0, st, a);         \
-        else hipLaunchKernelGGL((attn_bwd_dq_kernel<KS, NT, CAUSAL, 1>), dim3(grid_q), dim3(256), 0, st, a);                 \
-        int rc = check_launch("vaa_model_attention_bwd(dq)");                                                                \
-        if (rc != VAA_OK) return rc;                                                                                         \
-        if (gk == 2) hipLaunchKernelGGL((attn_bwd_dkv_kernel<KS, NT, CAUSAL, 2>), dim3(grid_k), dim3(256), 0, st, a);        \
-        else hipLaunchKernelGGL((attn_bwd_dkv_kernel<KS, NT, CAUSAL, 1>), dim3(grid_k), dim3(256), 0, st, a);                \
-        return check_launch("vaa_model_attention_bwd(dkv)");                                                                 \
-    } while (0)
-    if (a.hd <= 64) VAA_ATT_BWD(2, 4);
-    else if (a.hd <= 80) VAA_ATT_BWD(3, 5);
-    else if (a.hd <= 96) VAA_ATT_BWD(3, 6);
-    else VAA_ATT_BWD(4, 8);
-#undef VAA_ATT_BWD
-}
-
-template <bool CAUSAL>
+    if (ROPE) gq = gk = 1;
+    if (a.hd <= 64) return launch_bwd_t<2, 4, CAUSAL, ROPE>(a, gq, gk, st);
+    if (a.hd > 96) return launch_bwd_t<4, 8, CAUSAL, ROPE>(a, gq, gk, st);
+    if (a.hd <= 80) return launch_bwd_t<3, 5, CAUSAL, false>(a, gq, gk, st);
+    return launch_bwd_t<3, 6, CAUSAL, false>(a, gq, gk, st);
+}
+
+template <int KS, int NT, bool CAUSAL, bool ROPE>
+static int launch_fwd_t(const AttnFwdArgs& a, int gf, hipStream_t st) {
+    int sf, sq, sk;
+    attn_stages(a.hd, sf, sq, sk);
+    const unsigned grid = (unsigned)(((long)a.B * a.H + 7) / 8 * 8) * (unsigned)((a.T + kTile * gf - 1) / (kTile * gf));
+    VAA_ATT_PICK(attn_fwd_kernel, KS, NT, gf, sf, grid, a);
+    return check_launch("vaa_model_attention_fwd");
+}
+
+template <bool CAUSAL, bool ROPE>
 static int launch_fwd(const AttnFwdArgs& a, hipStream_t st) {
     int gf, gq, gk;
     attn_groups(a.hd, gf, gq, gk);
-    const unsigned grid = (unsigned)(((long)a.B * a.H + 7) / 8 * 8) * (unsigned)((a.T + kTile * gf - 1) / (kTile * gf));
-#define VAA_ATT_FWD(KS, NT)                                                                                          \
-    do {                                                                                                             \
-        if (gf == 2) hipLaunchKernelGGL((attn_fwd_kernel<KS, NT, CAUSAL, 2>), dim3(grid), dim3(256), 0, st, a);      \
-        else hipLaunchKernelGGL((attn_fwd_kernel<KS, NT, CAUSAL, 1>), dim3(grid), dim3(256), 0, st, a);              \
-    } while (0)
-    if (a.hd <= 64) VAA_ATT_FWD(2, 4);
-    else if (a.hd <= 80) VAA_ATT_FWD(3, 5);
-    else if (a.hd <= 96) VAA_ATT_FWD(3, 6);
-    else VAA_ATT_FWD(4, 8);
-#undef VAA_ATT_FWD
-    return check_launch("vaa_model_attention_fwd");
-}
+    if (ROPE) gf = 1;
+    if (a.hd <= 64) return launch_fwd_t<2, 4, CAUSAL, ROPE>(a, gf, st);
+    if (a.hd > 96) return launch_fwd_t<4, 8, CAUSAL, ROPE>(a, gf, st);
+    if (a.hd <= 80) return launch_fwd_t<3, 5, CAUSAL, false>(a, gf, st);
+    return launch_fwd_t<3, 6, CAUSAL, false>(a, gf, st);
+}
+#undef VAA_ATT_PICK
 
 static bool strides_ok(const int64_t* s) { return s && (s[0] % 8) == 0 && (s[1] % 8) == 0 && (s[2] % 8) == 0; }
 static AttnStr mk(const int64_t* s) { AttnStr r; r.b = s[0]; r.t = s[1]; r.h = s[2]; return r; }
 
 }
 
-extern "C" int vaa_model_attention_fwd(const uint16_t* q, const int64_t* q_str, const uint16_t* k, const int64_t* k_str, const uint16_t* v,
-                                       const int64_t* v_str, uint16_t* o, const int64_t* o_str, float* lse, const int32_t* cu_seqlens, int B,
-                                       int H, int T, int hd, int causal, float scale, void* stream) {
-    using namespace vaa;
+namespace vaa {
+
+static int attention_fwd(const char* who, const uint16_t* q, const int64_t* q_str, const uint16_t* k, const int64_t* k_str, const uint16_t* v,
+                         const int64_t* v_str, uint16_t* o, const int64_t* o_str, float* lse, const float* rope_cos, const float* rope_sin,
+                         const int32_t* cu_seqlens, int B, int H, int T, int hd, int causal, float scale, void* stream) {
     if (!q || !k || !v || !o || !lse) {
-        set_error("vaa_model_attention_fwd: null pointer argument");
+        set_error("%s: null pointer argument", who);
         return VAA_E_INVALID;
     }
     if (B <= 0 || H <= 0 || T <= 0 || hd <= 0 || hd > 128 || (hd % 8) != 0 || !strides_ok(q_str) || !strides_ok(k_str) || !strides_ok(v_str) ||
         !strides_ok(o_str)) {
-        set_error("vaa_model_attention_fwd: unsupported shape (B=%d H=%d T=%d hd=%d; hd %% 8 == 0, hd <= 128, strides %% 8 == 0)", B, H, T, hd);
+        set_error("%s: unsupported shape (B=%d H=%d T=%d hd=%d; hd %% 8 == 0, hd <= 128, strides %% 8 == 0)", who, B, H, T, hd);
         return VAA_E_UNSUPPORTED;
     }
     AttnFwdArgs a;
     a.q = q; a.k = k; a.v = v; a.o = o; a.lse = lse;
     a.sq = mk(q_str); a.sk = mk(k_str); a.sv = mk(v_str); a.so = mk(o_str);
     a.cu = cu_seqlens;
+    a.rope_cos = rope_cos; a.rope_sin = rope_sin;
     a.B = B; a.H = H; a.T = T; a.hd = hd;
     a.scale_log2 = scale * 1.4426950408889634f;
-    return causal ? launch_fwd<true>(a, (hipStream_t)stream) : launch_fwd<false>(a, (hipStream_t)stream);
+    const hipStream_t st = (hipStream_t)stream;
+    if (rope_cos) return causal ? launch_fwd<true, true>(a, st) : launch_fwd<false, true>(a, st);
+    return causal ? launch_fwd<true, false>(a, st) : launch_fwd<false, false>(a, st);
+}
+
+static int attention_bwd(const char* who, bool rope_in, const uint16_t* q, const int64_t* q_str, const uint16_t* k, const int64_t* k_str,
+                         const uint16_t* v, const int64_t* v_str, const uint16_t* o, const int64_t* o_str, const uint16_t* dout,
+                         const int64_t* do_str, const float* lse, float* dsum, uint16_t* dq, const int64_t* dq_str, uint16_t* dk,
+                         const int64_t* dk_str, uint16_t* dv, const int64_t* dv_str, const float* rope_cos, const float* rope_sin,
+                         const int32_t* cu_seqlens, int B, int H, int T, int hd, int causal, float scale, void* stream) {
+    if (!q || !k || !v || !o || !dout || !lse || !dsum || !dq || !dk || !dv) {
+        set_error("%s: null pointer argument", who);
+        return VAA_E_INVALID;
+    }
+    if (B <= 0 || H <= 0 || T <= 0 || hd <= 0 || hd > 128 || (hd % 8) != 0 || !strides_ok(q_str) || !strides_ok(k_str) || !strides_ok(v_str) ||
+        !strides_ok(o_str) || !strides_ok(do_str) || !strides_ok(dq_str) || !strides_ok(dk_str) || !strides_ok(dv_str)) {
+        set_error("%s: unsupported shape (B=%d H=%d T=%d hd=%d; hd %% 8 == 0, hd <= 128, strides %% 8 == 0)", who, B, H, T, hd);
+        return VAA_E_UNSUPPORTED;
+    }
+    AttnBwdArgs a;
+    a.q = q; a.k = k; a.v = v; a.o = o; a.dout = dout; a.lse = lse; a.dsum = dsum; a.dq = dq; a.dk = dk; a.dv = dv;
+    a.sq = mk(q_str); a.sk = mk(k_str); a.sv = mk(v_str); a.so = mk(o_str); a.sdo = mk(do_str);
+    a.sdq = mk(dq_str); a.sdk = mk(dk_str); a.sdv = mk(dv_str);
+    a.rope_cos = rope_cos; a.rope_sin = rope_sin;
+    a.cu = cu_seqlens;
+    a.B = B; a.H = H; a.T = T; a.hd = hd;
+    a.scale = scale;
+    a.scale_log2 = scale * 1.4426950408889634f;
+    const hipStream_t st = (hipStream_t)stream;
+    if (rope_in) return causal ? launch_bwd<true, true>(a, st) : launch_bwd<false, true>(a, st);
+    return causal ? launch_bwd<true, false>(a, st) : launch_bwd<false, false>(a, st);
+}
+
+static bool rope_tables_ok(const char* who, const float* rope_cos, const float* rope_sin, int hd, bool required) {
+    if ((rope_cos != nullptr) != (rope_sin != nullptr) || (required && !rope_cos) || (rope_cos && hd != 64 && hd != 128)) {
+        set_error("%s: the rotary embedding needs both tables and hd in {64, 128} (hd=%d)", who, hd);
+        return false;
+    }
+    return true;
+}
+
+}
+
+extern "C" int vaa_model_attention_form(int form) {
+    using namespace vaa;
+    if (form < 0) return attn_form().load();
+    return attn_form().exchange(form == kFormTile64 || form == kFormRopeIn ? form : (int)kFormCurrent);
+}
+
+extern "C" int vaa_model_attention_fwd(const uint16_t* q, const int64_t* q_str, const uint16_t* k, const int64_t* k_str, const uint16_t* v,
+                                       const int64_t* v_str, uint16_t* o, const int64_t* o_str, float* lse, const int32_t* cu_seqlens, int B,
+                                       int H, int T, int hd, int causal, float scale, void* stream) {
+    return vaa::attention_fwd("vaa_model_attention_fwd", q, q_str, k, k_str, v, v_str, o, o_str, lse, nullptr, nullptr, cu_seqlens, B, H, T, hd,
+                              causal, scale, stream);
+}
+
+extern "C" int vaa_model_attention_rope_fwd(const uint16_t* q, const int64_t* q_str, const uint16_t* k, const int64_t* k_str, const uint16_t* v,
+                                            const int64_t* v_str, uint16_t* o, const int64_t* o_str, float* lse, const float* rope_cos,
+                                            const float* rope_sin, const int32_t* cu_seqlens, int B, int H, int T, int hd, int causal, float scale,
+                                            void* stream) {
+    const char* who = "vaa_model_attention_rope_fwd";
+    if (!vaa::rope_tables_ok(who, rope_cos, rope_sin, hd, true)) return VAA_E_UNSUPPORTED;
+    return vaa::attention_fwd(who, q, q_str, k, k_str, v, v_str, o, o_str, lse, rope_cos, rope_sin, cu_seqlens, B, H, T, hd, causal, scale, stream);
 }
 
 extern "C" int vaa_model_attention_bwd(const uint16_t* q, const int64_t* q_str, const uint16_t* k, const int64_t* k_str, const uint16_t* v,
@@ -669,28 +885,20 @@
                                        const int64_t* do_str, const float* lse, float* dsum, uint16_t* dq, const int64_t* dq_str, uint16_t* dk,
                                        const int64_t* dk_str, uint16_t* dv, const int64_t* dv_str, const float* rope_cos, const float* rope_sin,
                                        const int32_t* cu_seqlens, int B, int H, int T, int hd, int causal, float scale, void* stream) {
-    using namespace vaa;
-    if (!q || !k || !v || !o || !dout || !lse || !dsum || !dq || !dk || !dv) {
-        set_error("vaa_model_attention_bwd: null pointer argument");
-        return VAA_E_INVALID;
-    }
-    if (B <= 0 || H <= 0 || T <= 0 || hd <= 0 || hd > 128 || (hd % 8) != 0 || !strides_ok(q_str) || !strides_ok(k_str) || !strides_ok(v_str) ||
-        !strides_ok(o_str) || !strides_ok(do_str) || !strides_ok(dq_str) || !strides_ok(dk_str) || !strides_ok(dv_str)) {
-        set_error("vaa_model_attention_bwd: unsupported shape (B=%d H=%d T=%d hd=%d; hd %% 8 == 0, hd <= 128, strides %% 8 == 0)", B, H, T, hd);
-        return VAA_E_UNSUPPORTED;
-    }
-    AttnBwdArgs a;
-    a.q = q; a.k = k; a.v = v; a.o = o; a.dout = dout; a.lse = lse; a.dsum = dsum; a.dq = dq; a.dk = dk; a.dv = dv;
-    a.sq = mk(q_str); a.sk = mk(k_str); a.sv = mk(v_str); a.so = mk(o_str); a.sdo = mk(do_str);
-    a.sdq = mk(dq_str); a.sdk = mk(dk_str); a.sdv = mk(dv_str);
-    if ((rope_cos != nullptr) != (rope_sin != nullptr) || (rope_cos && hd != 64 && hd != 128)) {
-        set_error("vaa_model_attention_bwd: fused rotary adjoint needs both tables and hd in {64, 128} (hd=%d)", hd);
-        return VAA_E_UNSUPPORTED;
-    }
-    a.rope_cos = rope_cos; a.rope_sin = rope_sin;
-    a.cu = cu_seqlens;
-    a.B = B; a.H = H; a.T = T; a.hd = hd;
-    a.scale = scale;
-    a.scale_log2 = scale * 1.4426950408889634f;
-    return causal ? launch_bwd<true>(a, (hipStream_t)stream) : launch_bwd<false>(a, (hipStream_t)stream);
-}
+    const char* who = "vaa_model_attention_bwd";
+    if (!vaa::rope_tables_ok(who, rope_cos, rope_sin, hd, false)) return VAA_E_UNSUPPORTED;
+    return vaa::attention_bwd(who, false, q, q_str, k, k_str, v, v_str, o, o_str, dout, do_str, lse, dsum, dq, dq_str, dk, dk_str, dv, dv_str,
+                              rope_cos, rope_sin, cu_seqlens, B, H, T, hd, causal, scale, stream);
+}
+
+extern "C" int vaa_model_attention_rope_bwd(const uint16_t* q, const int64_t* q_str, const uint16_t* k, const int64_t* k_str, const uint16_t* v,
+                                            const int64_t* v_str, const uint16_t* o, const int64_t* o_str, const uint16_t* dout,
+                                            const int64_t* do_str, const float* lse, float* dsum, uint16_t* dq, const int64_t* dq_str, uint16_t* dk,
+                                            const int64_t* dk_str, uint16_t* dv, const int64_t* dv_str, const float* rope_cos,
+                                            const float* rope_sin, const int32_t* cu_seqlens, int B, int H, int T, int hd, int causal, float scale,
+                                            void* stream) {
+    const char* who = "vaa_model_attention_rope_bwd";
+    if (!vaa::rope_tables_ok(who, rope_cos, rope_sin, hd, true)) return VAA_E_UNSUPPORTED;
+    return vaa::attention_bwd(who, true, q, q_str, k, k_str, v, v_str, o, o_str, dout, do_str, lse, dsum, dq, dq_str, dk, dk_str, dv, dv_str,
+                              rope_cos, rope_sin, cu_seqlens, B, H, T, hd, causal, scale, stream);
+}
diff --git a/roboticattack_amd/model_ops.py b/roboticattack_amd/model_ops.py
--- a/roboticattack_amd/model_ops.py
+++ b/roboticattack_amd/model_ops.py
@@ -195,20 +195,41 @@
     return (ctypes.c_int64 * 3)(x.stride(0), x.stride(1), x.stride(2))
 
 
-def attention_fwd(q: torch.Tensor, k: torch.Tensor, v: torch.Tensor, causal: bool, scale: float | None = None, cu_seqlens=None, max_len: int = 0):
+ATTENTION_FORMS = ("tile64", "current", "rope_in")
+
+
+def attention_form(form: str | None = None) -> str:
+    L = _lib.lib()
+    return ATTENTION_FORMS[L.vaa_model_attention_form(-1 if form is None else ATTENTION_FORMS.index(form))]
+
+
+def rope_in_kernel(hd: int) -> bool:
+    return hd in (64, 128) and attention_form() == "rope_in"
+
+
+def attention_fwd(q: torch.Tensor, k: torch.Tensor, v: torch.Tensor, causal: bool, scale: float | None = None, cu_seqlens=None, max_len: int = 0,
+                  rope=None):
     Bq, T, H, hd = q.shape
     scale = float(hd) ** -0.5 if scale is None else float(scale)
     o = torch.empty((Bq, T, H, hd), dtype=torch.bfloat16, device=q.device)
     B, Tm = (int(cu_seqlens.numel()) - 1, int(max_len)) if cu_seqlens is not None else (Bq, T)
     lse = torch.empty((B, H, Tm), dtype=torch.float32, device=q.device)
-    rc = _lib.lib().vaa_model_attention_fwd(q.data_ptr(), _str3(q), k.data_ptr(), _str3(k), v.data_ptr(), _str3(v), o.data_ptr(), _str3(o),
-                                            lse.data_ptr(), cu_seqlens.data_ptr() if cu_seqlens is not None else None, B, H, Tm, hd,
-                                            int(bool(causal)), scale, _stream())
-    _lib.check(rc, "vaa_model_attention_fwd")
+    cu = cu_seqlens.data_ptr() if cu_seqlens is not None else None
+    L = _lib.lib()
+    if rope is not None:
+        rc = L.vaa_model_attention_rope_fwd(q.data_ptr(), _str3(q), k.data_ptr(), _str3(k), v.data_ptr(), _str3(v), o.data_ptr(), _str3(o),
+                                            lse.data_ptr(), rope[0].data_ptr(), rope[1].data_ptr(), cu, B, H, Tm, hd, int(bool(causal)), scale,
+                                            _stream())
+        _lib.check(rc, "vaa_model_attention_rope_fwd")
+    else:
+        rc = L.vaa_model_attention_fwd(q.data_ptr(), _str3(q), k.data_ptr(), _str3(k), v.data_ptr(), _str3(v), o.data_ptr(), _str3(o),
+                                       lse.data_ptr(), cu, B, H, Tm, hd, int(bool(causal)), scale, _stream())
+        _lib.check(rc, "vaa_model_attention_fwd")
     return o, lse
 
 
-def attention_bwd(q, k, v, o, lse, dout, causal: bool, scale: float, packed_grad: bool = False, rope=None, cu_seqlens=None, max_len: int = 0):
+def attention_bwd(q, k, v, o, lse, dout, causal: bool, scale: float, packed_grad: bool = False, rope=None, cu_seqlens=None, max_len: int = 0,
+                  rope_in: bool = False):
     Bq, T, H, hd = q.shape
     B, Tm = (int(cu_seqlens.numel()) - 1, int(max_len)) if cu_seqlens is not None else (Bq, T)
     if dout.stride(3) != 1:
@@ -220,12 +241,15 @@
         buf = None
         dq, dk, dv = (torch.empty((Bq, T, H, hd), dtype=torch.bfloat16, device=q.device) for _ in range(3))
     dsum = torch.empty((B, H, Tm), dtype=torch.float32, device=q.device)
-    rc = _lib.lib().vaa_model_attention_bwd(q.data_ptr(), _str3(q), k.data_ptr(), _str3(k), v.data_ptr(), _str3(v), o.data_ptr(), _str3(o),
-                                            dout.data_ptr(), _str3(dout), lse.data_ptr(), dsum.data_ptr(), dq.data_ptr(), _str3(dq),
-                                            dk.data_ptr(), _str3(dk), dv.data_ptr(), _str3(dv), rope[0].data_ptr() if rope else None,
-                                            rope[1].data_ptr() if rope else None, cu_seqlens.data_ptr() if cu_seqlens is not None else None,
-                                            B, H, Tm, hd, int(bool(causal)), float(scale), _stream())
-    _lib.check(rc, "vaa_model_attention_bwd")
+    if rope_in and not rope:
+        raise ValueError("attention_bwd: rope_in needs the rotary tables")
+    fn = "vaa_model_attention_rope_bwd" if rope_in else "vaa_model_attention_bwd"
+    rc = getattr(_lib.lib(), fn)(q.data_ptr(), _str3(q), k.data_ptr(), _str3(k), v.data_ptr(), _str3(v), o.data_ptr(), _str3(o),
+                                 dout.data_ptr(), _str3(dout), lse.data_ptr(), dsum.data_ptr(), dq.data_ptr(), _str3(dq),
+                                 dk.data_ptr(), _str3(dk), dv.data_ptr(), _str3(dv), rope[0].data_ptr() if rope else None,
+                                 rope[1].data_ptr() if rope else None, cu_seqlens.data_ptr() if cu_seqlens is not None else None,
+                                 B, H, Tm, hd, int(bool(causal)), float(scale), _stream())
+    _lib.check(rc, fn)
     return buf if packed_grad else (dq, dk, dv)
 
 
@@ -251,17 +275,22 @@
     @staticmethod
     def forward(ctx, q, k, v, cos, sin, causal, scale, cu_seqlens=None, max_len=0):
         scale = float(q.shape[-1]) ** -0.5 if scale is None else float(scale)
-        qr, kr = _rope_launch(q, cos, sin, 1.0), _rope_launch(k, cos, sin, 1.0)
-        o, lse = attention_fwd(qr, kr, v, causal, scale, cu_seqlens, max_len)
-        ctx.save_for_backward(qr, kr, v, o, lse, cos, sin, *([cu_seqlens] if cu_seqlens is not None else []))
+        ctx.rope_in = rope_in_kernel(q.shape[-1])
+        if ctx.rope_in:
+            qs, ks = q, k
+            o, lse = attention_fwd(q, k, v, causal, scale, cu_seqlens, max_len, rope=(cos, sin))
+        else:
+            qs, ks = _rope_launch(q, cos, sin, 1.0), _rope_launch(k, cos, sin, 1.0)
+            o, lse = attention_fwd(qs, ks, v, causal, scale, cu_seqlens, max_len)
+        ctx.save_for_backward(qs, ks, v, o, lse, cos, sin, *([cu_seqlens] if cu_seqlens is not None else []))
         ctx.causal, ctx.scale, ctx.max_len = bool(causal), scale, int(max_len)
         return o
 
     @staticmethod
     def backward(ctx, dout):
-        qr, kr, v, o, lse, cos, sin, *cu = ctx.saved_tensors
-        dq, dk, dv = attention_bwd(qr, kr, v, o, lse, dout, ctx.causal, ctx.scale, rope=(cos, sin), cu_seqlens=cu[0] if cu else None,
-                                   max_len=ctx.max_len)
+        qs, ks, v, o, lse, cos, sin, *cu = ctx.saved_tensors
+        dq, dk, dv = attention_bwd(qs, ks, v, o, lse, dout, ctx.causal, ctx.scale, rope=(cos, sin), cu_seqlens=cu[0] if cu else None,
+                                   max_len=ctx.max_len, rope_in=ctx.rope_in)
         return dq, dk, dv, None, None, None, None, None, None
 
 
@@ -270,18 +299,26 @@
     @staticmethod
     def forward(ctx, qkv, cos, sin, causal, scale, cu_seqlens=None, max_len=0):
         scale = float(qkv.shape[-1]) ** -0.5 if scale is None else float(scale)
-        qr, kr = _rope_launch(qkv[:, :, 0], cos, sin, 1.0), _rope_launch(qkv[:, :, 1], cos, sin, 1.0)
         v = qkv[:, :, 2]
-        o, lse = attention_fwd(qr, kr, v, causal, scale, cu_seqlens, max_len)
-        ctx.save_for_backward(qr, kr, qkv, o, lse, cos, sin, *([cu_seqlens] if cu_seqlens is not None else []))
-        ctx.causal, ctx.scale, ctx.max_len = bool(causal), scale, int(max_len)
+        cu = [cu_seqlens] if cu_seqlens is not None else []
+        ctx.rope_in = rope_in_kernel(qkv.shape[-1])
+        if ctx.rope_in:
+            o, lse = attention_fwd(qkv[:, :, 0], qkv[:, :, 1], v, causal, scale, cu_seqlens, max_len, rope=(cos, sin))
+            ctx.save_for_backward(qkv, o, lse, cos, sin, *cu)
+        else:
+            qr, kr = _rope_launch(qkv[:, :, 0], cos, sin, 1.0), _rope_launch(qkv[:, :, 1], cos, sin, 1.0)
+            o, lse = attention_fwd(qr, kr, v, causal, scale, cu_seqlens, max_len)
+            ctx.save_for_backward(qkv, o, lse, cos, sin, *cu, qr, kr)
+        ctx.causal, ctx.scale, ctx.max_len, ctx.has_cu = bool(causal), scale, int(max_len), cu_seqlens is not None
         return o
 
     @staticmethod
     def backward(ctx, dout):
-        qr, kr, qkv, o, lse, cos, sin, *cu = ctx.saved_tensors
-        buf = attention_bwd(qr, kr, qkv[:, :, 2], o, lse, dout, ctx.causal, ctx.scale, packed_grad=True, rope=(cos, sin),
-                            cu_seqlens=cu[0] if cu else None, max_len=ctx.max_len)
+        qkv, o, lse, cos, sin, *rest = ctx.saved_tensors
+        cu = rest.pop(0) if ctx.has_cu else None
+        qs, ks = (qkv[:, :, 0], qkv[:, :, 1]) if ctx.rope_in else rest
+        buf = attention_bwd(qs, ks, qkv[:, :, 2], o, lse, dout, ctx.causal, ctx.scale, packed_grad=True, rope=(cos, sin),
+                            cu_seqlens=cu, max_len=ctx.max_len, rope_in=ctx.rope_in)
         return buf, None, None, None, None, None, None
 
 
```

Result: no change. 2.178 attack-steps/s, median of 6 (-0.0%).
